# declare-lab/tango

Hardware: AMD Instinct MI355X
Metric: audio-seconds generated/sec, Tango-full 200-step, batch=32, guidance=3 (higher is better)
Workload: dtype fp16; 1 GPU; BASELINE config 3: Tango-full UNet (866M) 200-step DDPM CFG=3 denoise + mel-VAE decode + HiFi-GAN, 32 prompts/GPU x 64 tokens; global_batch=32, text_len=64, denoise_steps=200, parallelism=dp1, rccl_ranks=1, hipgraph=True, fp8_attention=False

## Files before the change

include/tango_engine.h:

```cpp
#ifndef TANGO_ENGINE_H
#define TANGO_ENGINE_H

#include <stdint.h>

#ifdef __cplusplus
extern "C" {
#endif

#define TANGO_DTYPE_F32 0
#define TANGO_DTYPE_F16 1
#define TANGO_DTYPE_BF16 2

#define TANGO_PRED_EPSILON 0
#define TANGO_PRED_SAMPLE 1
#define TANGO_PRED_V 2

#define TANGO_RULE_DDPM 0
#define TANGO_RULE_DDIM 1
#define TANGO_RULE_DPM_MULTISTEP 2

#define TANGO_MAX_LEVELS 8

typedef struct tango_engine tango_engine_t;

// ... 36 lines not shown
  int32_t unet_attn_fp8;
} tango_config_t;

typedef struct tango_denoise_args {
  float* latents;
  const float* prompt_embeds;
  const uint8_t* prompt_mask;
  int32_t batch;
  int32_t text_len;
  int32_t num_steps;
  const int64_t* timesteps;
  const float* coef;
  float guidance_scale;
  int32_t prediction_type;
  int32_t rule;
  int32_t clip_sample;
  float clip_sample_range;
  const float* noise;
  uint64_t seed;
  int32_t sample_offset;
  int32_t use_graph;
  const float* beat_embeds;
  const uint8_t* beat_mask;
  int32_t beat_len;
  const float* chord_embeds;
  const uint8_t* chord_mask;
  int32_t chord_len;
  const uint8_t* prompt_mask_host;
  int32_t coef_width;
  const float* known_latents;
  const float* latent_mask;
  const float* blend_coef;
  const float* blend_noise;
} tango_denoise_args_t;

const char* tango_last_error(void);
const char* tango_version(void);

int tango_engine_create(const tango_config_t* cfg, tango_engine_t** out);
void tango_engine_destroy(tango_engine_t* h);

int tango_engine_num_weights(tango_engine_t* h);
const char* tango_engine_weight_name(tango_engine_t* h, int i);
int tango_engine_set_weight(tango_engine_t* h, const char* name, const float* dev_ptr, const int64_t* shape, int ndim);
int tango_engine_finalize_weights(tango_engine_t* h);

int tango_engine_denoise(tango_engine_t* h, const tango_denoise_args_t* args, void* stream);

int tango_engine_unet_forward(tango_engine_t* h, const float* sample, int64_t timestep, const float* prompt_embeds,
                              const uint8_t* prompt_mask, float* out, int batch2, int text_len, void* stream);

int tango_engine_unet_forward_music(tango_engine_t* h, const float* sample, int64_t timestep, const float* prompt_embeds,
                                    const uint8_t* prompt_mask, const float* beat_embeds, const uint8_t* beat_mask,
                                    const float* chord_embeds, const uint8_t* chord_mask, float* out, int batch2, int text_len,
                                    int beat_len, int chord_len, void* stream);

int tango_engine_vae_decode(tango_engine_t* h, const float* latents, float* mel, int batch, void* stream);
int tango_engine_vae_encode(tango_engine_t* h, const float* mel, float* moments, int batch, void* stream);
int tango_engine_vocode(tango_engine_t* h, const float* mel, int16_t* wav, int batch, int mel_frames, int* n_samples, void* stream);
int tango_engine_vocoder_samples(tango_engine_t* h, int mel_frames);

int tango_engine_encode_text(tango_engine_t* h, const int64_t* input_ids, const uint8_t* attention_mask, float* out, int batch,
                             int text_len, void* stream);

int tango_engine_mel_frames(tango_engine_t* h, int n_samples);
int tango_engine_mel_spectrogram(tango_engine_t* h, const float* wav, float* mel, float* log_magnitudes, float* energy, int batch,
                                 int n_samples, int* n_frames, void* stream);

int tango_engine_last_denoise_ms(tango_engine_t* h, float* total_ms, float* per_step_ms);
int tango_engine_last_step_gflop(tango_engine_t* h, double* gflop);

int tango_engine_set_plan_budget(tango_engine_t* h, uint64_t bytes);
int tango_engine_plan_stats(tango_engine_t* h, uint64_t* bytes_in_use, int* plans);
int tango_engine_drop_plans(tango_engine_t* h);

int tango_engine_profile_unet(tango_engine_t* h, int batch2, int text_len, char* report, int report_cap, void* stream);
int tango_engine_profile_vae(tango_engine_t* h, int batch, char* report, int report_cap, void* stream);
int tango_engine_profile_vocoder(tango_engine_t* h, int batch, int frames, char* report, int report_cap, void* stream);
void tango_tuning_reload(void);
const char* tango_debug_linear_route(int dtype, int M, int N, int K, int geglu, int ln_fold, int residual, int vt);

int tango_op_conv2d(int dtype, const float* x, const float* w, const float* bias, float* out, int B, int Cin, int H, int W,
                    int Cout, int stride, int upsample, void* stream);
int tango_op_linear(int dtype, const float* x, const float* w, const float* bias, const float* residual, float* out, int M,
                    int N, int K, int a_act, int e_act, int geglu, void* stream);
int tango_op_linear_ln(int dtype, const float* x, const float* w, const float* bias, const float* gamma, const float* beta,
                       const float* residual, float* out, int M, int N, int K, int geglu, float eps, void* stream);
int tango_op_linear_qkv(int dtype, const float* x, const float* w, const float* gamma, const float* beta, float* out_qk,
                        float* out_vt, int B, int S, int C, int K, float eps, void* stream);
int tango_op_linear_qkv_perm(int dtype, const float* x, const float* w, const float* gamma, const float* beta, float* out_qk,
                             float* out_vt, int B, int S, int C, int K, float eps, int vt_perm, void* stream);
int tango_op_ff_fused(int dtype, const float* x, const float* w1, const float* b1, const float* gamma, const float* beta, const float* w2,
                      const float* b2, float* out, int M, int C, int H, float eps, int mode, int reps, float* ms_out, void* stream);
int tango_op_qkv_stat(int dtype, const float* x, const float* w, const float* gamma, const float* beta, float* out_qk, float* out_vt, int B,
                      int S, int C, float eps, int mode, int reps, float* ms_out, void* stream);
int tango_op_conv1d(int dtype, const float* x, const float* w, const float* bias, const float* residual, float* out, int B,
                    int Cin, int L, int Cout, int k, int dilation, int a_act, float a_slope, int e_act, float e_slope, void* stream);
int tango_op_conv_transpose1d(int dtype, const float* x, const float* w, const float* bias, float* out, int B, int Cin, int L,
                              int Cout, int k, int stride, int padding, int a_act, float a_slope, void* stream);
int tango_op_groupnorm(int dtype, const float* x, const float* gamma, const float* beta, float* out, int B, int C, int HW,
                       int groups, float eps, int act, void* stream);
int tango_op_layernorm(int dtype, const float* x, const float* gamma, const float* beta, float* out, int rows, int C, float eps,
                       void* stream);
int tango_op_attention(int dtype, const float* q, const float* k, const float* v, const float* bias, float* out, int B, int heads,
                       int Sq, int Skv, float scale, void* stream);
int tango_op_attention_ex(int dtype, const float* q, const float* k, const float* v, const float* bias, float* out, int B, int heads,
                          int Sq, int Skv, float scale, int flags, void* stream);
int tango_op_xattn_block(int dtype, const float* x, const float* gamma, const float* beta, const float* wq, const float* k, const float* v,
                         const float* bias, const float* wo, const float* bo, float* out, int B, int HW, int L, float eps, void* stream);
int tango_op_sched_step(float* latents, const float* model_out_nchw, const float* noise, const float* coef8, int B, int C, int HW,
                        int cfg, float guidance, int pred_type, int rule, int clip, float clip_range, void* stream);

int tango_op_sched_multistep(float* latents, const float* model_out_nchw, float* ring, const float* coef16, int step, int B, int C,
                             int HW, int cfg, float guidance, int pred_type, int algo, void* stream);

int tango_op_philox_normal(float* out, int B, int C, int HW, int step, uint64_t seed, int sample_offset, void* stream);

int tango_op_sched_masked(float* latents, const float* model_out_nchw, const float* noise, float* ring, const float* coef, int coef_width,
                          int step, int num_steps, const float* known_latents, const float* latent_mask, const float* blend_coef,
                          const float* blend_noise, uint64_t seed, int sample_offset, int B, int C, int HW, int cfg, float guidance,
                          int pred_type, int rule, void* stream);

int tango_op_philox_normal_blend(float* out, int B, int C, int HW, int step, uint64_t seed, int sample_offset, void* stream);

#ifdef __cplusplus
}
#endif
#endif
```

tango_amd/_lib.py:

```python
import ctypes as C
import os

_HERE = os.path.dirname(os.path.abspath(__file__))
LIB_PATH = os.path.join(_HERE, "lib", "libtango_hip.so")
MAX_LEVELS = 8

DTYPES = {"fp32": 0, "float32": 0, "f32": 0, "fp16": 1, "float16": 1, "f16": 1, "bf16": 2, "bfloat16": 2}
PRED = {"epsilon": 0, "sample": 1, "v_prediction": 2}
RULE = {"ddpm": 0, "ddim": 1, "dpmsolver": 2}


class TangoConfig(C.Structure):
    _fields_ = [
        ("dtype", C.c_int32),
        ("unet_levels", C.c_int32),
        ("unet_channels", C.c_int32 * MAX_LEVELS),
        ("unet_heads", C.c_int32 * MAX_LEVELS),
        ("unet_cross_attn", C.c_int32 * MAX_LEVELS),
        ("unet_layers_per_block", C.c_int32),
        ("unet_in_channels", C.c_int32),
        ("unet_out_channels", C.c_int32),
        ("unet_cross_dim", C.c_int32),
        ("unet_groups", C.c_int32),
        ("unet_eps", C.c_float),
        ("unet_flip_sin_to_cos", C.c_int32),
        ("unet_freq_shift", C.c_float),
        ("latent_h", C.c_int32),
        ("latent_w", C.c_int32),
        ("vae_levels", C.c_int32),
        ("vae_ch", C.c_int32),
        ("vae_ch_mult", C.c_int32 * MAX_LEVELS),
        ("vae_num_res_blocks", C.c_int32),
        ("vae_z_channels", C.c_int32),
        ("vae_embed_dim", C.c_int32),
        ("vae_out_ch", C.c_int32),
        ("vae_scale_factor", C.c_float),
        ("voc_n_ups", C.c_int32),
        ("voc_rates", C.c_int32 * MAX_LEVELS),
        ("voc_kernels", C.c_int32 * MAX_LEVELS),
        ("voc_initial_channel", C.c_int32),
        ("voc_num_mels", C.c_int32),
        ("voc_n_resblocks", C.c_int32),
        ("voc_res_kernels", C.c_int32 * 4),
        ("voc_res_dilations", (C.c_int32 * 4) * 4),
        ("t5_layers", C.c_int32),
        ("t5_d_model", C.c_int32),
        ("t5_d_kv", C.c_int32),
        ("t5_heads", C.c_int32),
        ("t5_d_ff", C.c_int32),
        ("t5_vocab", C.c_int32),
        ("t5_rel_buckets", C.c_int32),
        ("t5_rel_max_distance", C.c_int32),
        ("t5_eps", C.c_float),
        ("vae_encoder", C.c_int32),
        ("vae_in_channels", C.c_int32),
        ("stft_filter_length", C.c_int32),
        ("stft_hop_length", C.c_int32),
        ("stft_n_mel", C.c_int32),
        ("unet_music", C.c_int32),
        ("unet_attn_fp8", C.c_int32),
    ]


class DenoiseArgs(C.Structure):
    _fields_ = [
        ("latents", C.c_void_p),
        ("prompt_embeds", C.c_void_p),
        ("prompt_mask", C.c_void_p),
        ("batch", C.c_int32),
        ("text_len", C.c_int32),
        ("num_steps", C.c_int32),
        ("timesteps", C.c_void_p),
        ("coef", C.c_void_p),
        ("guidance_scale", C.c_float),
        ("prediction_type", C.c_int32),
        ("rule", C.c_int32),
        ("clip_sample", C.c_int32),
        ("clip_sample_range", C.c_float),
        ("noise", C.c_void_p),
        ("seed", C.c_uint64),
        ("sample_offset", C.c_int32),
        ("use_graph", C.c_int32),
        ("beat_embeds", C.c_void_p),
        ("beat_mask", C.c_void_p),
        ("beat_len", C.c_int32),
        ("chord_embeds", C.c_void_p),
        ("chord_mask", C.c_void_p),
        ("chord_len", C.c_int32),
        ("prompt_mask_host", C.c_void_p),
        ("coef_width", C.c_int32),
        ("known_latents", C.c_void_p),
        ("latent_mask", C.c_void_p),
        ("blend_coef", C.c_void_p),
        ("blend_noise", C.c_void_p),
    ]


SYMBOLS = [
    "tango_last_error", "tango_version", "tango_tuning_reload", "tango_debug_linear_route", "tango_engine_create", "tango_engine_destroy",
    "tango_engine_num_weights", "tango_engine_weight_name", "tango_engine_set_weight",
    "tango_engine_finalize_weights", "tango_engine_denoise", "tango_engine_unet_forward", "tango_engine_unet_forward_music",
    "tango_engine_vae_decode", "tango_engine_vae_encode", "tango_engine_vocode", "tango_engine_vocoder_samples", "tango_engine_encode_text",
    "tango_engine_mel_frames", "tango_engine_mel_spectrogram",
    "tango_engine_last_denoise_ms", "tango_engine_last_step_gflop", "tango_engine_profile_unet", "tango_engine_profile_vae", "tango_engine_profile_vocoder", "tango_engine_set_plan_budget", "tango_engine_plan_stats", "tango_engine_drop_plans", "tango_op_conv2d", "tango_op_linear", "tango_op_linear_ln", "tango_op_ff_fused", "tango_op_qkv_stat", "tango_op_linear_qkv", "tango_op_linear_qkv_perm", "tango_op_conv1d",
    "tango_op_conv_transpose1d", "tango_op_groupnorm", "tango_op_layernorm", "tango_op_attention", "tango_op_attention_ex", "tango_op_xattn_block",
    "tango_op_sched_step", "tango_op_sched_multistep", "tango_op_philox_normal",
    "tango_op_sched_masked", "tango_op_philox_normal_blend",
]

_lib = None


def load():
    global _lib
    if _lib is not None:
        return _lib
    if not os.path.exists(LIB_PATH):
        raise ImportError(
            "tango_amd: %s not found. Build it with `make -C tango_amd/csrc` "
            "(or __graft_entry__.build()); the engine has no CPU/PyTorch fallback." % LIB_PATH)
    lib = C.CDLL(LIB_PATH, mode=C.RTLD_GLOBAL)
    vp, ci, cf, i64 = C.c_void_p, C.c_int, C.c_float, C.c_int64
    lib.tango_last_error.restype = C.c_char_p
    lib.tango_version.restype = C.c_char_p
    lib.tango_tuning_reload.restype = None
    lib.tango_engine_create.argtypes = [C.POINTER(TangoConfig), C.POINTER(vp)]
    lib.tango_engine_destroy.argtypes = [vp]
    lib.tango_engine_destroy.restype = None
    lib.tango_engine_num_weights.argtypes = [vp]
    lib.tango_engine_weight_name.argtypes = [vp, ci]
    lib.tango_engine_weight_name.restype = C.c_char_p
    lib.tango_engine_set_weight.argtypes = [vp, C.c_char_p, vp, C.POINTER(i64), ci]
    lib.tango_engine_finalize_weights.argtypes = [vp]
    lib.tango_engine_denoise.argtypes = [vp, C.POINTER(DenoiseArgs), vp]
    lib.tango_engine_unet_forward.argtypes = [vp, vp, i64, vp, vp, vp, ci, ci, vp]
    lib.tango_engine_unet_forward_music.argtypes = [vp, vp, i64, vp, vp, vp, vp, vp, vp, vp, ci, ci, ci, ci, vp]
    lib.tango_engine_vae_decode.argtypes = [vp, vp, vp, ci, vp]
    lib.tango_engine_vae_encode.argtypes = [vp, vp, vp, ci, vp]
    lib.tango_engine_vocode.argtypes = [vp, vp, vp, ci, ci, C.POINTER(ci), vp]
    lib.tango_engine_vocoder_samples.argtypes = [vp, ci]
    lib.tango_engine_encode_text.argtypes = [vp, vp, vp, vp, ci, ci, vp]
    lib.tango_engine_mel_frames.argtypes = [vp, ci]
    lib.tango_engine_mel_spectrogram.argtypes = [vp, vp, vp, vp, vp, ci, ci, C.POINTER(ci), vp]
    lib.tango_engine_last_denoise_ms.argtypes = [vp, C.POINTER(cf), C.POINTER(cf)]
    lib.tango_engine_last_step_gflop.argtypes = [vp, C.POINTER(C.c_double)]
    lib.tango_engine_profile_unet.argtypes = [vp, ci, ci, C.c_char_p, ci, vp]
    lib.tango_engine_profile_vae.argtypes = [vp, ci, C.c_char_p, ci, vp]
    lib.tango_engine_profile_vocoder.argtypes = [vp, ci, ci, C.c_char_p, ci, vp]
    lib.tango_engine_set_plan_budget.argtypes = [vp, C.c_uint64]
    lib.tango_engine_drop_plans.argtypes = [vp]
    lib.tango_debug_linear_route.argtypes = [ci] * 8
    lib.tango_debug_linear_route.restype = C.c_char_p
    lib.tango_engine_plan_stats.argtypes = [vp, C.POINTER(C.c_uint64), C.POINTER(ci)]
    lib.tango_op_conv2d.argtypes = [ci, vp, vp, vp, vp, ci, ci, ci, ci, ci, ci, ci, vp]
    lib.tango_op_linear.argtypes = [ci, vp, vp, vp, vp, vp, ci, ci, ci, ci, ci, ci, vp]
    lib.tango_op_linear_ln.argtypes = [ci, vp, vp, vp, vp, vp, vp, vp, ci, ci, ci, ci, cf, vp]
    lib.tango_op_ff_fused.argtypes = [ci, vp, vp, vp, vp, vp, vp, vp, vp, ci, ci, ci, cf, ci, ci, vp, vp]
    lib.tango_op_qkv_stat.argtypes = [ci, vp, vp, vp, vp, vp, vp, ci, ci, ci, cf, ci, ci, vp, vp]
    lib.tango_op_linear_qkv.argtypes = [ci, vp, vp, vp, vp, vp, vp, ci, ci, ci, ci, cf, vp]
    lib.tango_op_linear_qkv_perm.argtypes = [ci, vp, vp, vp, vp, vp, vp, ci, ci, ci, ci, cf, ci, vp]
    lib.tango_op_conv1d.argtypes = [ci, vp, vp, vp, vp, vp, ci, ci, ci, ci, ci, ci, ci, cf, ci, cf, vp]
    lib.tango_op_conv_transpose1d.argtypes = [ci, vp, vp, vp, vp, ci, ci, ci, ci, ci, ci, ci, ci, cf, vp]
    lib.tango_op_groupnorm.argtypes = [ci, vp, vp, vp, vp, ci, ci, ci, ci, cf, ci, vp]
    lib.tango_op_layernorm.argtypes = [ci, vp, vp, vp, vp, ci, ci, cf, vp]
    lib.tango_op_attention.argtypes = [ci, vp, vp, vp, vp, vp, ci, ci, ci, ci, cf, vp]
    lib.tango_op_attention_ex.argtypes = [ci, vp, vp, vp, vp, vp, ci, ci, ci, ci, cf, ci, vp]
    lib.tango_op_xattn_block.argtypes = [ci, vp, vp, vp, vp, vp, vp, vp, vp, vp, vp, ci, ci, ci, cf, vp]
    lib.tango_op_sched_step.argtypes = [vp, vp, vp, vp, ci, ci, ci, ci, cf, ci, ci, ci, cf, vp]
    lib.tango_op_sched_multistep.argtypes = [vp, vp, vp, vp, ci, ci, ci, ci, ci, cf, ci, ci, vp]
    lib.tango_op_philox_normal.argtypes = [vp, ci, ci, ci, ci, C.c_uint64, ci, vp]
    lib.tango_op_philox_normal_blend.argtypes = [vp, ci, ci, ci, ci, C.c_uint64, ci, vp]
    lib.tango_op_sched_masked.argtypes = [vp, vp, vp, vp, vp, ci, ci, ci, vp, vp, vp, vp, C.c_uint64, ci, ci, ci, ci, ci, cf, ci, ci, vp]
    _lib = lib
    return lib


def check(rc, what="tango engine call"):
    if rc != 0:
        msg = load().tango_last_error()
        msg = msg.decode() if msg else "unknown error"
        if "cannot be larger" in msg or "unknown prediction" in msg:
            raise ValueError(msg)
        raise RuntimeError("%s failed: %s" % (what, msg))
```

tango_amd/csrc/common.h:

```cpp
#pragma once
#include <hip/hip_runtime.h>
#include <stdint.h>
#include <string>

namespace tango {

enum DType : int { DT_F32 = 0, DT_F16 = 1, DT_BF16 = 2 };

typedef _Float16 f16;
typedef __bf16 bf16;
typedef float f32x4 __attribute__((ext_vector_type(4)));
typedef float f32x2 __attribute__((ext_vector_type(2)));
typedef _Float16 f16x8 __attribute__((ext_vector_type(8)));
typedef _Float16 f16x4 __attribute__((ext_vector_type(4)));
typedef __bf16 bf16x8 __attribute__((ext_vector_type(8)));
typedef __bf16 bf16x4 __attribute__((ext_vector_type(4)));
typedef unsigned u32x4 __attribute__((ext_vector_type(4)));
typedef unsigned u32x2 __attribute__((ext_vector_type(2)));

inline size_t dtype_size(int dt) { return dt == DT_F32 ? 4 : 2; }

template <typename T> struct TypeTag;
template <> struct TypeTag<float> { static constexpr int dt = DT_F32; };
template <> struct TypeTag<f16> { static constexpr int dt = DT_F16; };
// ... 26 lines not shown
template <typename T> __device__ __forceinline__ float to_f(T v) { return (float)v; }
template <typename T> __device__ __forceinline__ T from_f(float v) { return (T)v; }

__device__ __forceinline__ float silu_f(float x) { return x / (1.0f + __expf(-x)); }
__device__ __forceinline__ float gelu_erf_f(float x) { return 0.5f * x * (1.0f + erff(x * 0.70710678118654752440f)); }
__device__ __forceinline__ float gelu_tanh_f(float x) {
  return 0.5f * x * (1.0f + tanhf(0.7978845608028654f * (x + 0.044715f * x * x * x)));
}
typedef float f32x2_t __attribute__((ext_vector_type(2)));
__device__ __forceinline__ f32x2_t gelu_erf_poly2(const f32x2_t x) {
  f32x2_t xc;
  xc.x = __builtin_amdgcn_fmed3f(x.x, -4.25f, 4.25f);
  xc.y = __builtin_amdgcn_fmed3f(x.y, -4.25f, 4.25f);
  const f32x2_t t = xc * xc;
  f32x2_t q = f32x2_t{1.498029197e-11f, 1.498029197e-11f} + t * 1.123676848e-12f;
  q = __builtin_elementwise_fma(q, t, f32x2_t{-7.180728823e-09f, -7.180728823e-09f});
  q = __builtin_elementwise_fma(q, t, f32x2_t{3.825664002e-07f, 3.825664002e-07f});
  q = __builtin_elementwise_fma(q, t, f32x2_t{-1.045047183e-05f, -1.045047183e-05f});
  q = __builtin_elementwise_fma(q, t, f32x2_t{1.811638670e-04f, 1.811638670e-04f});
  q = __builtin_elementwise_fma(q, t, f32x2_t{-2.193588131e-03f, -2.193588131e-03f});
  q = __builtin_elementwise_fma(q, t, f32x2_t{1.957916536e-02f, 1.957916536e-02f});
  q = __builtin_elementwise_fma(q, t, f32x2_t{-1.326353318e-01f, -1.326353318e-01f});
  q = __builtin_elementwise_fma(q, t, f32x2_t{7.977887478e-01f, 7.977887478e-01f});
  const f32x2_t e = q * xc, h = x * 0.5f;
  return __builtin_elementwise_fma(h, e, h);
}
template <typename T, typename V4> __device__ __forceinline__ void glu_gate4(V4& v, const float g[4], int tanh_form) {
  if (tanh_form) {
#pragma unroll
    for (int r = 0; r < 4; ++r) v[r] = v[r] * gelu_tanh_f(g[r]);
  } else if constexpr (sizeof(T) == 4) {
#pragma unroll
    for (int r = 0; r < 4; ++r) v[r] = v[r] * gelu_erf_f(g[r]);
  } else {
    const f32x2_t a = gelu_erf_poly2(f32x2_t{g[0], g[1]}), b = gelu_erf_poly2(f32x2_t{g[2], g[3]});
    v[0] = v[0] * a.x; v[1] = v[1] * a.y; v[2] = v[2] * b.x; v[3] = v[3] * b.y;
  }
}

enum Act : int { ACT_NONE = 0, ACT_SILU = 1, ACT_LRELU = 2, ACT_GELU = 3, ACT_TANH = 4, ACT_GELU_TANH = 5 };

__device__ __forceinline__ float apply_act(float x, int act, float slope) {
  switch (act) {
    case ACT_SILU: return silu_f(x);
    case ACT_LRELU: return x > 0.f ? x : x * slope;
    case ACT_GELU: return gelu_erf_f(x);
    case ACT_TANH: return tanhf(x);
    case ACT_GELU_TANH: return gelu_tanh_f(x);
    default: return x;
  }
}

template <typename V4> __device__ __forceinline__ void apply_act4(V4& v, int act, float slope) {
  if (act == ACT_LRELU) {
#pragma unroll
    for (int r = 0; r < 4; ++r) v[r] = v[r] > 0.f ? v[r] : v[r] * slope;
  } else if (act == ACT_SILU) {
#pragma unroll
    for (int r = 0; r < 4; ++r) v[r] = silu_f(v[r]);
  } else if (act == ACT_TANH) {
#pragma unroll
    for (int r = 0; r < 4; ++r) v[r] = tanhf(v[r]);
  } else if (act == ACT_GELU) {
#pragma unroll
    for (int r = 0; r < 4; ++r) v[r] = gelu_erf_f(v[r]);
  } else if (act == ACT_GELU_TANH) {
#pragma unroll
    for (int r = 0; r < 4; ++r) v[r] = gelu_tanh_f(v[r]);
  }
}

struct View {
  void* p = nullptr;
  int64_t ld = 0;
  int C = 0;
};

enum GatherMode : int { GATHER_1D = 0, GATHER_2D = 1 };
enum Epi : int { EPI_NONE = 0, EPI_GEGLU = 1, EPI_I16 = 2, EPI_VT = 3 };

struct GemmParams {
  const void* A = nullptr;
  const void* W = nullptr;
  const float* bias = nullptr;
  const float* bias2 = nullptr;
  const int* step_ptr = nullptr;
  int bias2_stride = 0;
  const void* R = nullptr;
  int64_t ldr = 0;
  void* out = nullptr;
  int64_t ldo = 0;
  int out_f32 = 0;
  int M = 0, N = 0, K = 0, Cin = 0;
  int64_t Kp = 0;
  int64_t lda = 0;
  int stage_epi = 0;
  int mode = GATHER_1D;
  int H = 0, Wd = 0, Hin = 0, Win = 0, stride = 1, ups = 0;
  int pad = 1;
  int rows_pb = 0, Lin = 0, taps = 1, tap_step = 1, in_off = 0, in_mul = 1;
  int Lout = 0, out_mul = 1, out_off = 0;
  int a_act = ACT_NONE;
  float a_slope = 0.f;
  int epi = EPI_NONE;
  int glu_tanh = 0;
  int e_act = ACT_NONE;
  float e_slope = 0.f;
  float alpha = 1.f;
  float out_scale = 1.f;
  int bias_rows = 0;
  void* vt = nullptr;
  int vt_n0 = 0, vt_S = 1;
  int64_t vt_ld = 0;
  int vt_perm = 0;
  const float* rowvec = nullptr;
  int64_t rowvec_rows = 0;
  int rowvec_per = 1;
  void* out_lo = nullptr;
  int64_t ldo_lo = 0;
  int64_t wb_stride = 0;
  int wb_rows = 0;
  int ln_fold = 0;
  float ln_eps = 1e-5f;
  const float* wsum = nullptr;
  const float* row_stats = nullptr;
  int splitk = 1;
  float* ws = nullptr;
  int batch = 1;
  int64_t sA = 0, sW = 0, sO = 0, sR = 0, sBias = 0;
};

int launch_gemm(int dtype, const GemmParams& p, hipStream_t s);
enum GemmRoute : int { ROUTE_NONE = 0, ROUTE_WIDE, ROUTE_STREAM, ROUTE_CONV_WIDE, ROUTE_CONV_HALO, ROUTE_DMA, ROUTE_TILE, ROUTE_DUO };
int gemm_route(int dtype, const GemmParams& p);
bool gemm_rowvec_ok(int dtype, const GemmParams& p);
bool conv_halo_ok(int dtype, const GemmParams& p);
int launch_conv_halo(int dtype, const GemmParams& p, const unsigned char* zero_page, hipStream_t s);
bool gemm_wide_ok(int dtype, const GemmParams& p);
int launch_gemm_wide(int dtype, const GemmParams& p, hipStream_t s);
int gemm_wide_pers_cus();
bool gemm_duo_ok(int dtype, const GemmParams& p);
int launch_gemm_duo(int dtype, const GemmParams& p, hipStream_t s);
inline bool gemm_ln_fold_ok(int dtype, const GemmParams& p);
bool conv_wide_ok(int dtype, const GemmParams& p);
int launch_conv_wide(int dtype, const GemmParams& p, const unsigned char* zero_page, hipStream_t s);
int conv_wide_pick_splitk(int dtype, const GemmParams& p);
int launch_splitk_reduce(int dtype, const GemmParams& p, hipStream_t s);
bool gemm_dma_ok(int dtype, const GemmParams& p);
int launch_gemm_dma(int dtype, const GemmParams& p, const unsigned char* zero_page, hipStream_t s);
int gemm_init();
int gemm_pick_splitk(int dtype, const GemmParams& p);
bool linear_stream_ok(int dtype, const GemmParams& p);
int launch_linear_stream(int dtype, const GemmParams& p, hipStream_t s);
inline bool gemm_ln_fold_ok(int dtype, const GemmParams& p) { return linear_stream_ok(dtype, p) || gemm_wide_ok(dtype, p) || gemm_duo_ok(dtype, p); }
int launch_fold_ln(int dtype, const void* W, int64_t Kp, const float* gamma, const float* beta, const float* bias_in, void* Wo,
                   float* bias_out, float* wsum, int N, int K, hipStream_t s);

struct FFParams {
  const void* x = nullptr; int64_t ldx = 0;
  const void* w1 = nullptr; int64_t ld1 = 0;
  const float* b1 = nullptr;
  const void* w2 = nullptr; int64_t ld2 = 0;
  const float* b2 = nullptr;
  void* out = nullptr; int64_t ldo = 0;
  int M = 0, C = 0, H = 0;
  float eps = 1e-5f;
  int plain_loop = 0;
};
bool ff_fused_ok(int dtype, const FFParams& p);
int launch_ff_fused(int dtype, const FFParams& p, hipStream_t s);

struct QKVParams {
  const void* x = nullptr; int64_t ldx = 0;
  const void* w = nullptr; int64_t ldw = 0;
  const float* b = nullptr;
  void* out = nullptr; int64_t ldo = 0;
  void* vt = nullptr; int64_t vt_ld = 0; int vt_S = 0;
  int vt_perm = 0;
  int M = 0, N = 0, K = 0, n_rm = 0;
  int ln = 1; float eps = 1e-5f;
  const float* gstats = nullptr;
  int groups = 0, rows_ps = 0;
};
bool qkv_stat_ok(int dtype, const QKVParams& p);
int launch_qkv_stat(int dtype, const QKVParams& p, hipStream_t s);

struct GroupNormParams {
  const void* x; int64_t ldx;
  void* y; int64_t ldy;
  const float* gamma; const float* beta;
  int B, rows, C, groups;
  float eps;
  int act;
  float* partial;
  float* scale_shift;
  unsigned* sync = nullptr;
};
constexpr int COOP_SYNC_SLOTS = 1024;
constexpr int coop_sync_words() { return 2 * COOP_SYNC_SLOTS + 16; }
size_t groupnorm_ws_floats(int B, int rows, int C, int groups);
int launch_gn_stats_fold(int dtype, const GroupNormParams& p, const void* W, int64_t Kp, const float* bias, int N, void* Wf, float* bf, hipStream_t s);
bool gn_fold_ok(int dtype, const GroupNormParams& p, int N);
bool gn_stats_mr_ok(int dtype, const GroupNormParams& p);
int launch_gn_stats_mr(int dtype, const GroupNormParams& p, float* mr, hipStream_t s);
int launch_groupnorm(int dtype, const GroupNormParams& p, hipStream_t s);

int launch_layernorm(int dtype, const void* x, int64_t ldx, void* y, int64_t ldy, const float* gamma,
                     const float* beta, int rows, int C, float eps, hipStream_t s);
int launch_ln_stats(int dtype, const void* x, int64_t ldx, float* stats, int rows, int C, float eps, hipStream_t s);

struct AttnParams {
  const void* q; int64_t ldq;
  const void* k; int64_t ldk;
  const void* vt; int64_t ldvt;
  void* o; int64_t ldo;
  const float* bias;
  const float* pos_bias = nullptr;
  int B, heads, Sq, Skv;
  float scale;
  int vt_perm = 0;
  int fp8_pv = 0;
};
int launch_attention(int dtype, const AttnParams& p, hipStream_t s);
__host__ __device__ inline int vt_perm_pos(int s) { return (s & ~31) | ((s & 12) << 1) | ((s & 16) >> 2) | (s & 3); }
bool attention_vt_perm_ok(int dtype, const AttnParams& p);

struct XAttnParams {
  const void* x; int64_t ldx;
  const void* wq;
// ... 76 lines not shown
```

tango_amd/csrc/conv_wide.hip:

```cpp
#include <cstdlib>
#include <type_traits>

#include "common.h"
#include "tuning.h"
#include "gemm_device.h"
#include "gemm_wide_device.h"

namespace tango {

static constexpr int CW_HALO_MAX = 544;
static constexpr int CW_NA_WIDE = 5;
static constexpr int CW_NA = CW_NA_WIDE;
static constexpr int CW_HALO_MAX_TALL = 800;
static constexpr int CW_NA_TALL = 7;

template <typename T, bool RES, bool SK, int SCH, bool TALL>
__global__ __launch_bounds__(512) void conv3x3_wide_kernel(const GemmParams p, const unsigned char* zero_page, const int SR, const int nseg,
                                                           const int abytes, const int prio) {
  constexpr int BM = TALL ? 512 : 256, BN = TALL ? 160 : 320, CB = 64, NST = 4;
  constexpr int CW_NA = TALL ? CW_NA_TALL : CW_NA_WIDE;
  constexpr int BK = CB / (int)sizeof(T);
  constexpr int WST = BN * CB;
  constexpr int WRG = BN / 16;
  constexpr int WRGW = (WRG + 7) / 8;
  constexpr int TM = 4, TN = 10;
  extern __shared__ __attribute__((aligned(16))) unsigned char dsm[];
  unsigned char* const As = dsm;
  unsigned char* const Ws = dsm + 2 * abytes;

  const int NT = p.N / BN;
  int bid = blockIdx.x;
  {
    const int nblk = gridDim.x, q = nblk >> 3, r = nblk & 7, xcd = bid & 7, idx = bid >> 3;
    bid = (xcd < r ? xcd * (q + 1) : r * (q + 1) + (xcd - r) * q) + idx;
  }
  const int m0 = (bid / NT) * BM, n0 = (bid % NT) * BN;
  const unsigned char* Ab = (const unsigned char*)p.A;
  const unsigned char* Wb = (const unsigned char*)p.W;
  const int tid = threadIdx.x, lane = tid & 63;
  const int wave = __builtin_amdgcn_readfirstlane(tid >> 6);
  const int wm = TALL ? wave : wave & 3, wn = TALL ? 0 : wave >> 2;
  const int lrow = lane >> 2, slot = lane & 3;

  const int H = p.H, Wd = p.Wd, hw = H * Wd;
  const int HW2 = Wd + 2, SEG = (SR + 2) * HW2;
  const int HALO = nseg * SEG, HALO_RG = (HALO + 15) >> 4;
  const int b0 = m0 / hw;
  const int y0 = nseg == 1 ? (m0 - b0 * hw) / Wd : 0;

  unsigned* const aoff_lds = (unsigned*)(Ws + NST * WST) + tid;
#pragma unroll
  for (int t = 0; t < CW_NA; ++t) {
    unsigned off = ~0u;
    const int h = ((t * 8 + wave) << 4) + lrow;
    if (h < HALO) {
      const int seg = h / SEG, rem = h - seg * SEG;
      const int hy = rem / HW2, hx = rem - hy * HW2;
      const int y = y0 + hy - 1, x = hx - 1;
      const int pc = slot ^ ((h >> 1) & 2);
      if ((unsigned)y < (unsigned)H && (unsigned)x < (unsigned)Wd)
        off = (unsigned)(((((int64_t)(b0 + seg) * p.Hin + (y >> p.ups)) * p.Win + (x >> p.ups)) * p.lda) * (int64_t)sizeof(T) + pc * 16);
    }
    aoff_lds[t * 512] = off;
  }
  const int wrow_d = wave * 16 + lrow;
  const unsigned w_off0_init = (unsigned)(((int64_t)wrow_d * p.Kp) * (int64_t)sizeof(T) + ((slot ^ ((wrow_d >> 1) & 2)) * 16));
  aoff_lds[CW_NA * 512] = w_off0_init;
  const unsigned w_step = (unsigned)(128 * p.Kp * (int64_t)sizeof(T));
  const unsigned char* const Wt = Wb + (int64_t)n0 * p.Kp * (int64_t)sizeof(T);
  const int my_w = wave < WRG - 8 * (WRGW - 1) ? WRGW : WRGW - 1;

  auto issue_a_off = [&](const int t, const int cc, const int buf, const unsigned off) {
    const unsigned char* src = off != ~0u ? Ab + (int64_t)cc * CB + off : zero_page;
    __builtin_amdgcn_global_load_lds((gptr_t)src, (lptr_t)(As + buf * abytes + (t * 8 + wave) * 1024), 16, 0, 0);
  };
  auto issue_a = [&](const int t, const int cc, const int buf) {
    if (t * 8 + wave < HALO_RG) issue_a_off(t, cc, buf, aoff_lds[t * 512]);
  };
  auto issue_w_one = [&](const int i, int koff, const int st, const unsigned w_off0) {
    const int rg = wave + 8 * i;
    if (rg < WRG) {
      asm volatile("" : "+s"(koff));
      const unsigned char* base = Wt + koff;
      unsigned o = w_off0 + i * w_step;
      asm volatile("" : "+v"(o));
      __builtin_amdgcn_global_load_lds((gptr_t)(base + o), (lptr_t)(Ws + st * WST + rg * 1024), 16, 0, 0);
    }
  };
  auto issue_w = [&](const int tap, const int cc, const int st) {
    const int koff = (tap * p.Cin + cc * BK) * (int)sizeof(T);
    const unsigned w_off0 = aoff_lds[CW_NA * 512];
#pragma unroll
    for (int i = 0; i < WRGW; ++i) issue_w_one(i, koff, st, w_off0);
  };
  auto wait_n = [&](const int n) {
    switch (n) {
      case 0: wait_vmcnt_lit<0>(); break;
      case 1: wait_vmcnt_lit<1>(); break;
      case 2: wait_vmcnt_lit<2>(); break;
      case 3: wait_vmcnt_lit<3>(); break;
      case 4: wait_vmcnt_lit<4>(); break;
      case 5: wait_vmcnt_lit<5>(); break;
      case 6: wait_vmcnt_lit<6>(); break;
      case 7: wait_vmcnt_lit<7>(); break;
      default: wait_vmcnt_lit<8>(); break;
    }
  };

  f32x4 acc[TN][TM];
#pragma unroll
  for (int a = 0; a < TN; ++a)
#pragma unroll
    for (int b = 0; b < TM; ++b) acc[a][b] = f32x4{0.f, 0.f, 0.f, 0.f};

  int h0 = 0, hd[TM];
#pragma unroll
  for (int b = 0; b < TM; ++b) {
    const int pm = wm * 64 + b * 16 + (lane & 15);
    const int seg = pm / hw, r = pm - seg * hw;
    const int ly = r / Wd, x = r - ly * Wd;
    const int hb_ = seg * SEG + ly * HW2 + x;
    if (b == 0) h0 = hb_;
    hd[b] = __builtin_amdgcn_readfirstlane(hb_ - h0);
  }
  const int kg = lane >> 4;
  const int wrow0 = wn * (TN * 16) + (lane & 15);
  const int wfoff = wrow0 * CB + ((kg ^ ((wrow0 >> 1) & 2)) << 4);

  int cc0 = 0, cc1 = p.Cin / BK;
  if (SK) {
    const int per = (cc1 + (int)gridDim.y - 1) / (int)gridDim.y;
    cc0 = (int)blockIdx.y * per;
    cc1 = cc1 < cc0 + per ? cc1 : cc0 + per;
  }
  const int NI = (cc1 - cc0) * 9;

  const int half = wave >> 2;
#pragma unroll
  for (int t = 0; t < CW_NA; ++t) issue_a(t, cc0, cc0 & 1);
  issue_w(0, cc0, 0);
  issue_w(1, cc0, 1);
  issue_w(2, cc0, 2);
  wait_n(2 * my_w);
  pp_barrier();
  if (half) pp_barrier();
  if (prio == 2 && half) __builtin_amdgcn_s_setprio(1);
  int st = 0, item = 0;
  int prev_h = 0;
  unsigned hoff = 0u;
  unsigned w_off0 = w_off0_init;
  asm volatile("" : "+v"(w_off0));
  for (int cc = cc0; cc < cc1; ++cc) {
    const unsigned char* Ah = As + (cc & 1) * abytes;
    const bool more_c = cc + 1 < cc1;
#pragma unroll 1
    for (int tap = 0; tap < 9; ++tap, ++item) {
      const unsigned char* Wst = Ws + st * WST;
      const int toff = (tap / 3) * HW2 + (tap % 3);
      const bool iss_h = more_c && tap < CW_NA && tap * 8 + wave < HALO_RG;
      const bool iss_w = item + 3 < NI;
      const int st3 = st == 0 ? 3 : st - 1;
      int koff3;
      {
        int t3 = tap + 3, c3 = cc;
        if (t3 >= 9) { t3 -= 9; c3 = cc + 1; }
        koff3 = (t3 * p.Cin + c3 * BK) * (int)sizeof(T);
      }
      if (SCH != 0) { if (iss_h) hoff = aoff_lds[tap * 512]; }
      u32x4 wf[TN], xf[TM];
#pragma unroll
      for (int a = 0; a < TN; ++a) wf[a] = *(const u32x4*)(Wst + wfoff + a * 16 * CB);
#pragma unroll
      for (int b = 0; b < TM; ++b) {
        int hs = hd[b] + toff;
        asm volatile("" : "+s"(hs));
        const int h = h0 + hs;
        xf[b] = *(const u32x4*)(Ah + h * CB + ((kg ^ ((h >> 1) & 2)) << 4));
      }
      if (item + 1 < NI) wait_n(prev_h + (item + 2 < NI ? my_w : 0));
      prev_h = iss_h ? 1 : 0;
      pp_barrier();
      if (SCH == 0) {
        if (more_c && tap < CW_NA) issue_a(tap, cc + 1, (cc + 1) & 1);
        const int t3 = tap + 3;
        if (t3 < 9) issue_w(t3, cc, st3);
        else if (more_c) issue_w(t3 - 9, cc + 1, st3);
      }
      if (prio == 0) __builtin_amdgcn_s_setprio(1);
#pragma unroll
      for (int a = 0; a < TN; ++a) {
#pragma unroll
        for (int b = 0; b < TM; ++b) Mma<T>::run(acc[a][b], wf[a], xf[b]);
        if (SCH != 0 && (a & 1) == 0 && (a >> 1) <= WRGW) {
          const int sl = a >> 1;
          __builtin_amdgcn_sched_barrier(0);
          if (sl == 0) { if (iss_h) issue_a_off(tap, cc + 1, (cc + 1) & 1, hoff); }
          else if (iss_w) issue_w_one(sl - 1, koff3, st3, w_off0);
          __builtin_amdgcn_sched_barrier(0);
        }
      }
      if (prio == 0) __builtin_amdgcn_s_setprio(0);
      pp_barrier();
      st = st == NST - 1 ? 0 : st + 1;
    }
  }
  if (!half) pp_barrier();
  if (prio == 2) __builtin_amdgcn_s_setprio(0);
  __syncthreads();
  unsigned char* const slice = dsm + wave * (WIDE_STAGE_BYTES + 1280);
  if (SK) {
    wide_epilogue_raw(p, acc, (int)blockIdx.y, m0 + wm * 64, n0 + wn * (TN * 16), lane, slice);
    return;
  }
  const float mean[TM] = {0.f, 0.f, 0.f, 0.f}, rstd[TM] = {1.f, 1.f, 1.f, 1.f};
  wide_epilogue<T, false, RES, false>(p, acc, mean, rstd, m0 + wm * 64, n0 + wn * (TN * 16), lane, slice);
}

template <int OFF> __device__ __forceinline__ void cwp_lds_read(u32x4& v, const unsigned base) {
  asm volatile("ds_read_b128 %0, %1 offset:%2" : "=v"(v) : "v"(base), "n"(OFF));
}
__device__ __forceinline__ void cwp_lds_wait_all(u32x4 (&wf)[10], u32x4 (&xf)[4], unsigned& hoff) {
  asm volatile("s_waitcnt lgkmcnt(0)"
               : "+v"(wf[0]), "+v"(wf[1]), "+v"(wf[2]), "+v"(wf[3]), "+v"(wf[4]), "+v"(wf[5]), "+v"(wf[6]), "+v"(wf[7]), "+v"(wf[8]), "+v"(wf[9]),
                 "+v"(xf[0]), "+v"(xf[1]), "+v"(xf[2]), "+v"(xf[3]), "+v"(hoff));
}
__device__ __forceinline__ void cwp_lds_read_b32(unsigned& v, const unsigned addr) { asm volatile("ds_read_b32 %0, %1" : "=v"(v) : "v"(addr)); }
template <int I, int N, typename F> __device__ __forceinline__ void cwp_for(F&& f) {
  if constexpr (I < N) { f(std::integral_constant<int, I>{}); cwp_for<I + 1, N>(f); }
}

template <typename T, bool RES, bool SK, int MODE = 0>
__global__ __launch_bounds__(512) void conv3x3_wide_pipe_kernel(const GemmParams p, const unsigned char* zero_page, const int SR, const int nseg,
                                                                const int abytes, const int prio) {
  constexpr bool LOCK = MODE == 1, SKEW = MODE == 2;
  constexpr int BM = 256, BN = 320, CB = 64, NST = 4;
  constexpr int BK = CB / (int)sizeof(T);
  constexpr int WST = BN * CB;
  constexpr int WRG = BN / 16;
  constexpr int WRGW = (WRG + 7) / 8;
  constexpr int TM = 4, TN = 10;
  extern __shared__ __attribute__((aligned(16))) unsigned char dsm[];
  unsigned char* const As = dsm;
  unsigned char* const Ws = dsm + 2 * abytes;

  const int NT = p.N / BN;
  int bid = blockIdx.x;
  {
    const int nblk = gridDim.x, q = nblk >> 3, r = nblk & 7, xcd = bid & 7, idx = bid >> 3;
    bid = (xcd < r ? xcd * (q + 1) : r * (q + 1) + (xcd - r) * q) + idx;
  }
  const int m0 = (bid / NT) * BM, n0 = (bid % NT) * BN;
  const unsigned char* Ab = (const unsigned char*)p.A;
  const unsigned char* Wb = (const unsigned char*)p.W;
  const int tid = threadIdx.x, lane = tid & 63;
  const int wave = __builtin_amdgcn_readfirstlane(tid >> 6);
  const int wm = wave & 3, wn = wave >> 2;
  const int lrow = lane >> 2, slot = lane & 3;

  const int H = p.H, Wd = p.Wd, hw = H * Wd;
  const int HW2 = Wd + 2, SEG = (SR + 2) * HW2;
  const int HALO = nseg * SEG, HALO_RG = (HALO + 15) >> 4;
  const int b0 = m0 / hw;
  const int y0 = nseg == 1 ? (m0 - b0 * hw) / Wd : 0;

  unsigned* const aoff_lds = (unsigned*)(Ws + NST * WST) + tid;
#pragma unroll
  for (int t = 0; t < CW_NA; ++t) {
    unsigned off = ~0u;
    const int h = ((t * 8 + wave) << 4) + lrow;
    if (h < HALO) {
      const int seg = h / SEG, rem = h - seg * SEG;
      const int hy = rem / HW2, hx = rem - hy * HW2;
      const int y = y0 + hy - 1, x = hx - 1;
      const int pc = slot ^ ((h >> 1) & 2);
      if ((unsigned)y < (unsigned)H && (unsigned)x < (unsigned)Wd)
        off = (unsigned)(((((int64_t)(b0 + seg) * p.Hin + (y >> p.ups)) * p.Win + (x >> p.ups)) * p.lda) * (int64_t)sizeof(T) + pc * 16);
    }
    aoff_lds[t * 512] = off;
  }
  const int wrow_d = wave * 16 + lrow;
  const unsigned w_off0_init = (unsigned)(((int64_t)wrow_d * p.Kp) * (int64_t)sizeof(T) + ((slot ^ ((wrow_d >> 1) & 2)) * 16));
  const unsigned w_step = (unsigned)(128 * p.Kp * (int64_t)sizeof(T));
  const unsigned char* const Wt = Wb + (int64_t)n0 * p.Kp * (int64_t)sizeof(T);
  const int my_w = wave < WRG - 8 * (WRGW - 1) ? WRGW : WRGW - 1;

  auto issue_a_off = [&](const int t, const int cc, const int buf, const unsigned off) {
    const unsigned char* src = off != ~0u ? Ab + (int64_t)cc * CB + off : zero_page;
    __builtin_amdgcn_global_load_lds((gptr_t)src, (lptr_t)(As + buf * abytes + (t * 8 + wave) * 1024), 16, 0, 0);
  };
  auto issue_w_one = [&](const int i, int koff, const int st, const unsigned w_off0) {
    const int rg = wave + 8 * i;
    if (rg < WRG) {
      asm volatile("" : "+s"(koff));
      const unsigned char* base = Wt + koff;
      unsigned o = w_off0 + i * w_step;
      asm volatile("" : "+v"(o));
      __builtin_amdgcn_global_load_lds((gptr_t)(base + o), (lptr_t)(Ws + st * WST + rg * 1024), 16, 0, 0);
    }
// ... 173 lines not shown
    unsigned xa[TM];
#pragma unroll
    for (int b = 0; b < TM; ++b) xa[b] = MORE1 ? xaddr(b, buf1, toff1) : 0u;
    cwp_for<0, TM>([&](auto b_tag) {
      constexpr int b = decltype(b_tag)::value;
      Mma<T>::run(acc[9][b], wf[9], xf[b]);
      __builtin_amdgcn_sched_barrier(0);
      if (MORE1) cwp_lds_read<0>(xf[b], xa[b]);
      if constexpr (2 + b <= WRGW) { if (half) dma_slot(std::integral_constant<int, 2 + b>{}); }
      __builtin_amdgcn_sched_barrier(0);
    });
    if (MORE1) {
      cwp_lds_read<9 * 16 * CB>(wf[9], wsrc);
      cwp_lds_read_b32(hoff, aoff_addr + (unsigned)(tap1 < CW_NA ? tap1 : 0) * 2048u);
      cwp_lds_wait_all(wf, xf, hoff);
    }
    return iss_h ? 1 : 0;
  };
  auto run_items = [&](auto item_fn) __attribute__((always_inline)) {
    int tap = 0, cc = cc0, prev_h = 0;
    unsigned hoff = hoff0;
#pragma unroll 1
    for (int item = 0; item + 1 < NI; ++item) {
      prev_h = item_fn(std::true_type{}, item, tap, cc, prev_h, hoff);
      if (tap == 8) { tap = 0; ++cc; } else ++tap;
    }
    item_fn(std::false_type{}, NI - 1, 8, cc1 - 1, prev_h, hoff);
  };
  if constexpr (SKEW) run_items(do_item_skew);
  else run_items(do_item);
  if (MODE == 0 && !half) pp_barrier();
  if (prio == 2) __builtin_amdgcn_s_setprio(0);
  __syncthreads();
  unsigned char* const slice = dsm + wave * (WIDE_STAGE_BYTES + 1280);
  if (SK) {
    wide_epilogue_raw(p, acc, (int)blockIdx.y, m0 + wm * 64, n0 + wn * (TN * 16), lane, slice);
    return;
  }
  const float mean[TM] = {0.f, 0.f, 0.f, 0.f}, rstd[TM] = {1.f, 1.f, 1.f, 1.f};
  wide_epilogue<T, false, RES, false>(p, acc, mean, rstd, m0 + wm * 64, n0 + wn * (TN * 16), lane, slice);
}

struct WideHaloGeom {
  int SR, nseg, halo;
};

static bool wide_halo_geom(const GemmParams& p, WideHaloGeom& g, const int BM = 256) {
  const int hw = p.H * p.Wd;
  if (p.Wd <= 0 || BM % p.Wd != 0) return false;
  if (hw >= BM) {
    if (hw % BM != 0) return false;
    g.SR = BM / p.Wd; g.nseg = 1;
  } else {
    if (BM % hw != 0) return false;
    g.SR = p.H; g.nseg = BM / hw;
  }
  g.halo = g.nseg * (g.SR + 2) * (p.Wd + 2);
  if (!((16 % p.Wd == 0 || p.Wd % 16 == 0) && hw % 16 == 0)) return false;
  return g.halo <= (BM == 512 ? CW_HALO_MAX_TALL : CW_HALO_MAX);
}

static bool conv_wide_tall_ok(const GemmParams& p) {
  if (!tuning().conv_tall || p.splitk > 1 || p.M % 512 != 0) return false;
  WideHaloGeom g;
  return wide_halo_geom(p, g, 512);
}

bool conv_wide_ok(int dtype, const GemmParams& p) {
  if (tuning().no_wide_conv || dtype == DT_F32) return false;
  if (p.mode != GATHER_2D || p.stride != 1 || p.pad != 1 || p.ups < 0 || p.ups > 1 || (p.Hin << p.ups) != p.H || (p.Win << p.ups) != p.Wd) return false;
  if (p.batch != 1 || p.a_act != ACT_NONE || p.epi != EPI_NONE || p.bias_rows) return false;
  if (p.splitk > 1 ? (!p.ws || p.splitk > p.Cin / 32 || p.N % 4 != 0) : (p.e_act != ACT_NONE || p.out_f32)) return false;
  if ((p.Cin * 2) % 64 != 0 || p.K != 9 * p.Cin || p.M % 256 != 0 || p.N % 320 != 0) return false;
  if (p.ldo % 8 != 0 || ((uintptr_t)p.out & 15) || (p.R && (p.ldr % 8 != 0 || ((uintptr_t)p.R & 15)))) return false;
  if ((p.lda * 2) % 16 != 0 || (p.Kp * 2) % 16 != 0 || ((uintptr_t)p.A & 15) || ((uintptr_t)p.W & 15)) return false;
  if (((uintptr_t)p.bias & 15) || ((uintptr_t)p.bias2 & 15) || (p.bias2 && p.bias2_stride % 4 != 0)) return false;
  if ((int64_t)(p.M >> (2 * p.ups)) * p.lda * 2 >= (int64_t)0xFFFF0000 || (int64_t)320 * p.Kp * 2 >= (int64_t)0xFFFF0000) return false;
  WideHaloGeom g;
  if (!wide_halo_geom(p, g)) return false;
  const long tiles = (long)(p.M / 256) * (p.N / 320) * (p.splitk > 1 ? p.splitk : 1);
  return tuning().force_big_kernels || tiles >= 224;
}

int conv_wide_pick_splitk(int dtype, const GemmParams& p) {
  GemmParams q = p;
  q.splitk = 1;
  if (tuning().force_big_kernels || p.mode != GATHER_2D || dtype == DT_F32 || p.M % 256 != 0 || p.N % 320 != 0 || p.Cin % 32 != 0) return 0;
  const long tiles = (long)(p.M / 256) * (p.N / 320);
  if (tiles > 96 || tiles < 16) return 0;
  int s = (int)((256 + tiles / 2) / tiles);
  const int nc = p.Cin / 32;
  if (s > nc / 4) s = nc / 4;
  if (s < 2) return 0;
  float dummy_ws = 0.f;
  q.splitk = s; q.ws = &dummy_ws;
  return conv_wide_ok(dtype, q) ? s : 0;
}

template <typename T, bool RES, bool SK, int SCH, bool TALL = false>
static int launch_conv_wide_sch(const GemmParams& p, const unsigned char* zero_page, hipStream_t s) {
  constexpr int BM = TALL ? 512 : 256, BN = TALL ? 160 : 320, NA = TALL ? CW_NA_TALL : CW_NA_WIDE;
  WideHaloGeom g;
  if (!wide_halo_geom(p, g, BM)) TANGO_FAIL("conv_wide: unsupported geometry");
  const int abytes = ((g.halo + 15) / 16) * 1024;
  int lds = 2 * abytes + 4 * BN * 64 + (NA + 1) * 512 * 4;
  const int epi_lds = 8 * (WIDE_STAGE_BYTES + 1280);
  if (lds < epi_lds) lds = epi_lds;
  auto kfn = conv3x3_wide_kernel<T, RES, SK, SCH, TALL>;
  TANGO_TRY(ensure_dyn_lds(reinterpret_cast<const void*>(kfn), lds));
  const int tiles = (p.M / BM) * (p.N / BN);
  hipLaunchKernelGGL(kfn, dim3((unsigned)tiles, (unsigned)(p.splitk > 1 ? p.splitk : 1)), dim3(512), lds, s, p, zero_page, g.SR, g.nseg, abytes, tuning().wide_prio);
  TANGO_HIP(hipGetLastError());
  if (p.splitk > 1) TANGO_TRY(launch_splitk_reduce(TypeTag<T>::dt, p, s));
  return 0;
}

template <typename T, bool RES, bool SK>
static int launch_conv_wide_pipe(const GemmParams& p, const unsigned char* zero_page, hipStream_t s) {
  WideHaloGeom g;
  if (!wide_halo_geom(p, g)) TANGO_FAIL("conv_wide: unsupported geometry");
  const int abytes = ((g.halo + 15) / 16) * 1024;
  int lds = 2 * abytes + 4 * 320 * 64 + (CW_NA + 1) * 512 * 4;
  const int epi_lds = 8 * (WIDE_STAGE_BYTES + 1280);
  if (lds < epi_lds) lds = epi_lds;
  const int mode = tuning().conv_pipe;
  auto kfn = mode == 3 ? conv3x3_wide_pipe_kernel<T, RES, SK, 2> : mode == 2 ? conv3x3_wide_pipe_kernel<T, RES, SK, 1> : conv3x3_wide_pipe_kernel<T, RES, SK, 0>;
  TANGO_TRY(ensure_dyn_lds(reinterpret_cast<const void*>(kfn), lds));
  const int tiles = (p.M / 256) * (p.N / 320);
  hipLaunchKernelGGL(kfn, dim3((unsigned)tiles, (unsigned)(p.splitk > 1 ? p.splitk : 1)), dim3(512), lds, s, p, zero_page, g.SR, g.nseg, abytes, tuning().wide_prio);
  TANGO_HIP(hipGetLastError());
  if (p.splitk > 1) TANGO_TRY(launch_splitk_reduce(TypeTag<T>::dt, p, s));
  return 0;
}

template <typename T, bool RES, bool SK = false>
static int launch_conv_wide_cfg(const GemmParams& p, const unsigned char* zero_page, hipStream_t s) {
  if (tuning().conv_pipe && !(SK ? false : conv_wide_tall_ok(p))) return launch_conv_wide_pipe<T, RES, SK>(p, zero_page, s);
  if constexpr (!SK) {
    if (conv_wide_tall_ok(p)) return launch_conv_wide_sch<T, RES, false, 1, true>(p, zero_page, s);
  }
  switch (tuning().wide_sched) {
    case 0: return launch_conv_wide_sch<T, RES, SK, 0>(p, zero_page, s);
    default: return launch_conv_wide_sch<T, RES, SK, 1>(p, zero_page, s);
  }
}

int launch_conv_wide(int dtype, const GemmParams& p, const unsigned char* zero_page, hipStream_t s) {
  if (!zero_page) TANGO_FAIL("conv_wide: gemm_init() was not called (zero page for the LDS-DMA gather)");
  switch (dtype) {
    case DT_F16:
      if (p.splitk > 1) return launch_conv_wide_cfg<f16, false, true>(p, zero_page, s);
      return p.R ? launch_conv_wide_cfg<f16, true>(p, zero_page, s) : launch_conv_wide_cfg<f16, false>(p, zero_page, s);
    case DT_BF16:
      if (p.splitk > 1) return launch_conv_wide_cfg<bf16, false, true>(p, zero_page, s);
      return p.R ? launch_conv_wide_cfg<bf16, true>(p, zero_page, s) : launch_conv_wide_cfg<bf16, false>(p, zero_page, s);
  }
  TANGO_FAIL("conv_wide: 16-bit dtypes only");
}

}
```

tango_amd/csrc/elementwise.hip:

```cpp
#include "common.h"

namespace tango {

__device__ __forceinline__ void philox4x32(unsigned c0, unsigned c1, unsigned c2, unsigned c3, unsigned k0, unsigned k1,
                                           unsigned* out) {
#pragma unroll
  for (int r = 0; r < 10; ++r) {
    const unsigned long long p0 = (unsigned long long)0xD2511F53u * c0;
    const unsigned long long p1 = (unsigned long long)0xCD9E8D57u * c2;
    const unsigned n0 = (unsigned)(p1 >> 32) ^ c1 ^ k0;
    const unsigned n1 = (unsigned)p1;
    const unsigned n2 = (unsigned)(p0 >> 32) ^ c3 ^ k1;
    const unsigned n3 = (unsigned)p0;
    c0 = n0; c1 = n1; c2 = n2; c3 = n3;
    k0 += 0x9E3779B9u; k1 += 0xBB67AE85u;
  }
  out[0] = c0; out[1] = c1; out[2] = c2; out[3] = c3;
}

__device__ __forceinline__ void box_muller(unsigned a, unsigned b, float& n0, float& n1) {
  const float u1 = ((float)a + 1.0f) * 2.3283064365386963e-10f;
  const float u2 = (float)b * 2.3283064365386963e-10f;
  const float r = sqrtf(-2.0f * __logf(u1));
  float s, c;
// ... 372 lines not shown
                    float slope, hipStream_t s) {
  const int epv = dtype == DT_F32 ? 4 : 8;
  if (n % epv) TANGO_FAIL("avg3: n must be a multiple of the 16-byte vector");
  const int64_t nvec = n / epv;
  unsigned nb = (unsigned)((nvec + 255) / 256);
  if (nb > 8192) nb = 8192;
  switch (dtype) {
    case DT_F32: hipLaunchKernelGGL((avg3_act_kernel<float>), dim3(nb), dim3(256), 0, s, (const float*)a, (const float*)b, (const float*)c, (float*)y, nvec, scale, act, slope); break;
    case DT_F16: hipLaunchKernelGGL((avg3_act_kernel<f16>), dim3(nb), dim3(256), 0, s, (const f16*)a, (const f16*)b, (const f16*)c, (f16*)y, nvec, scale, act, slope); break;
    case DT_BF16: hipLaunchKernelGGL((avg3_act_kernel<bf16>), dim3(nb), dim3(256), 0, s, (const bf16*)a, (const bf16*)b, (const bf16*)c, (bf16*)y, nvec, scale, act, slope); break;
    default: TANGO_FAIL("avg3: bad dtype");
  }
  TANGO_HIP(hipGetLastError());
  return 0;
}

__global__ void mask_bias_kernel(const uint8_t* __restrict__ m, float* __restrict__ bias, int n) {
  const int i = blockIdx.x * 256 + threadIdx.x;
  if (i < n) bias[i] = (1.0f - (m[i] ? 1.0f : 0.0f)) * -10000.0f;
}
int launch_mask_bias(const uint8_t* mask, float* bias, int n, hipStream_t s) {
  hipLaunchKernelGGL(mask_bias_kernel, dim3((unsigned)((n + 255) / 256)), dim3(256), 0, s, mask, bias, n);
  TANGO_HIP(hipGetLastError());
  return 0;
}

__global__ void timestep_embedding_kernel(const int64_t* __restrict__ ts, float* __restrict__ out, int n, int dim, int flip,
                                          float freq_shift) {
  const int i = blockIdx.x, half = dim / 2;
  for (int j = threadIdx.x; j < half; j += blockDim.x) {
    const float ex = __fdiv_rn(__fmul_rn(-9.210340371976184f, (float)j), (float)half - freq_shift);
    const float arg = __fmul_rn((float)ts[i], expf(ex));
    const float sv = sinf(arg), cv = cosf(arg);
    if (flip) { out[(int64_t)i * dim + j] = cv; out[(int64_t)i * dim + half + j] = sv; }
    else { out[(int64_t)i * dim + j] = sv; out[(int64_t)i * dim + half + j] = cv; }
  }
  if ((dim & 1) && threadIdx.x == 0) out[(int64_t)i * dim + dim - 1] = 0.f;
}
int launch_timestep_embedding(const int64_t* ts_dev, float* out, int n, int dim, int flip, float freq_shift, hipStream_t s) {
  hipLaunchKernelGGL(timestep_embedding_kernel, dim3((unsigned)n), dim3(256), 0, s, ts_dev, out, n, dim, flip, freq_shift);
  TANGO_HIP(hipGetLastError());
  return 0;
}

__device__ __forceinline__ int geglu_row(int o, int half) {
  const int j = o < half ? o : o - half;
  return 32 * (j >> 4) + (j & 15) + (o < half ? 0 : 16);
}

template <typename T>
__global__ __launch_bounds__(256) void pack_kernel(const float* __restrict__ src, T* __restrict__ dst, int O, int Tn, int I,
                                                   int64_t so, int64_t st, int64_t si, int64_t Kp, int64_t row_off, int perm) {
  const int64_t idx = (int64_t)blockIdx.x * 256 + threadIdx.x;
  if (idx >= (int64_t)O * Kp) return;
  const int o = (int)(idx / Kp);
  const int k = (int)(idx - (int64_t)o * Kp);
  float v = 0.f;
  if (k < Tn * I) {
    const int t = k / I, i = k - t * I;
    v = src[(int64_t)o * so + (int64_t)t * st + (int64_t)i * si];
  }
  int orow = o;
  if (perm == 1) orow = geglu_row(o, O / 2);
  else if (perm == 2) orow = 32 * (o >> 4) + (o & 15);
  else if (perm == 3) orow = 32 * (o >> 4) + (o & 15) + 16;
  dst[(row_off + orow) * Kp + k] = from_f<T>(v);
}

int launch_pack(int dtype, const float* src, void* dst, int O, int Tn, int I, int64_t so, int64_t st, int64_t si, int64_t Kp,
                int64_t dst_row_off, hipStream_t s) {
  const int perm = dst_row_off < 0 ? (int)(-dst_row_off) : 0;
  const int64_t ro = perm ? 0 : dst_row_off;
  const unsigned nb = (unsigned)(((int64_t)O * Kp + 255) / 256);
  switch (dtype) {
    case DT_F32: hipLaunchKernelGGL((pack_kernel<float>), dim3(nb), dim3(256), 0, s, src, (float*)dst, O, Tn, I, so, st, si, Kp, ro, perm); break;
    case DT_F16: hipLaunchKernelGGL((pack_kernel<f16>), dim3(nb), dim3(256), 0, s, src, (f16*)dst, O, Tn, I, so, st, si, Kp, ro, perm); break;
    case DT_BF16: hipLaunchKernelGGL((pack_kernel<bf16>), dim3(nb), dim3(256), 0, s, src, (bf16*)dst, O, Tn, I, so, st, si, Kp, ro, perm); break;
    default: TANGO_FAIL("pack: bad dtype");
  }
  TANGO_HIP(hipGetLastError());
  return 0;
}


template <typename T>
__global__ __launch_bounds__(256) void pointwise_small_kernel(const float* __restrict__ src, const float* __restrict__ W,
                                                              const float* __restrict__ bias, T* __restrict__ dst, int64_t ld,
                                                              int B, int Cin, int Cout, int HW, float scale) {
  const int64_t idx = (int64_t)blockIdx.x * 256 + threadIdx.x;
  if (idx >= (int64_t)B * HW) return;
  const int b = (int)(idx / HW), hw = (int)(idx - (int64_t)b * HW);
  float x[16];
  for (int c = 0; c < Cin; ++c) x[c] = src[((int64_t)b * Cin + c) * HW + hw] * scale;
  for (int o = 0; o < Cout; ++o) {
    float a = bias ? bias[o] : 0.f;
    for (int c = 0; c < Cin; ++c) a += W[o * Cin + c] * x[c];
    dst[idx * ld + o] = from_f<T>(a);
  }
}
int launch_pointwise_small(int dtype, const float* src, const float* W, const float* b, void* dst, int64_t ld, int B, int Cin,
                           int Cout, int HW, float scale, hipStream_t s) {
  if (Cin > 16) TANGO_FAIL("pointwise_small: Cin > 16");
  const unsigned nb = (unsigned)(((int64_t)B * HW + 255) / 256);
  switch (dtype) {
    case DT_F32: hipLaunchKernelGGL((pointwise_small_kernel<float>), dim3(nb), dim3(256), 0, s, src, W, b, (float*)dst, ld, B, Cin, Cout, HW, scale); break;
    case DT_F16: hipLaunchKernelGGL((pointwise_small_kernel<f16>), dim3(nb), dim3(256), 0, s, src, W, b, (f16*)dst, ld, B, Cin, Cout, HW, scale); break;
    case DT_BF16: hipLaunchKernelGGL((pointwise_small_kernel<bf16>), dim3(nb), dim3(256), 0, s, src, W, b, (bf16*)dst, ld, B, Cin, Cout, HW, scale); break;
    default: TANGO_FAIL("pointwise_small: bad dtype");
  }
  TANGO_HIP(hipGetLastError());
  return 0;
}

__global__ __launch_bounds__(256) void pointwise_out_nchw_kernel(const float* __restrict__ src, int64_t ld, const float* __restrict__ W,
                                                                 const float* __restrict__ bias, float* __restrict__ dst, int B, int Cin,
                                                                 int Cout, int HW) {
  const int64_t idx = (int64_t)blockIdx.x * 256 + threadIdx.x;
  if (idx >= (int64_t)B * HW) return;
  const int b = (int)(idx / HW), hw = (int)(idx - (int64_t)b * HW);
  float x[32];
  for (int c = 0; c < Cin; ++c) x[c] = src[idx * ld + c];
  for (int o = 0; o < Cout; ++o) {
    float a = bias ? bias[o] : 0.f;
    for (int c = 0; c < Cin; ++c) a += W[o * Cin + c] * x[c];
    dst[((int64_t)b * Cout + o) * HW + hw] = a;
  }
}
int launch_pointwise_out_nchw(const float* src, int64_t ld, const float* W, const float* b, float* dst, int B, int Cin, int Cout, int HW,
                              hipStream_t s) {
  if (Cin > 32) TANGO_FAIL("pointwise_out_nchw: Cin > 32");
  const unsigned nb = (unsigned)(((int64_t)B * HW + 255) / 256);
  hipLaunchKernelGGL(pointwise_out_nchw_kernel, dim3(nb), dim3(256), 0, s, src, ld, W, b, dst, B, Cin, Cout, HW);
  TANGO_HIP(hipGetLastError());
  return 0;
}

__global__ void permute_geglu_bias_kernel(const float* __restrict__ src, float* __restrict__ dst, int n) {
  const int i = blockIdx.x * 256 + threadIdx.x;
  if (i < n) dst[geglu_row(i, n / 2)] = src[i];
}
int launch_permute_geglu_bias(const float* src, float* dst, int n, hipStream_t s) {
  hipLaunchKernelGGL(permute_geglu_bias_kernel, dim3((unsigned)((n + 255) / 256)), dim3(256), 0, s, src, dst, n);
  TANGO_HIP(hipGetLastError());
  return 0;
}

int launch_fill_zero(void* p, size_t bytes, hipStream_t s) {
  TANGO_HIP(hipMemsetAsync(p, 0, bytes, s));
  return 0;
}

int launch_linear_f32(const float*, const float*, const float*, float*, int, int, int, int, int, hipStream_t) {
  TANGO_FAIL("linear_f32: not implemented (use launch_gemm with DT_F32)");
}

template <typename T>
__global__ __launch_bounds__(256) void embed_gather_kernel(const int64_t* __restrict__ ids, const float* __restrict__ table,
                                                           T* __restrict__ out, int64_t ld, int rows, int D, int vocab) {
  const int r = blockIdx.x;
  int64_t id = ids[r];
  id = id < 0 ? 0 : (id >= vocab ? vocab - 1 : id);
  const float* src = table + id * D;
  T* dst = out + (int64_t)r * ld;
  for (int c = threadIdx.x * 4; c < D; c += 1024) {
    const f32x4 v = *(const f32x4*)(src + c);
    dst[c] = from_f<T>(v[0]); dst[c + 1] = from_f<T>(v[1]); dst[c + 2] = from_f<T>(v[2]); dst[c + 3] = from_f<T>(v[3]);
// ... 143 lines not shown
```

tango_amd/csrc/engine.h:

```cpp
#pragma once
#include <array>
#include <functional>
#include <map>
#include <memory>
#include <string>
#include <unordered_map>
#include <vector>

#include "../../include/tango_engine.h"
#include "common.h"

namespace tango {

using Op = std::function<int(hipStream_t)>;

struct Program {
  std::vector<Op> ops;
  std::vector<std::string> labels;
  std::vector<double> flops;
  int run(hipStream_t s) const {
    for (const auto& o : ops) TANGO_TRY(o(s));
    return 0;
  }
  int run_profiled(hipStream_t s, std::string& report) const;
};

struct Arena {
  char* base = nullptr;
  size_t off = 0, peak = 0;
  void* alloc(size_t bytes) {
    off = (off + 255) & ~(size_t)255;
    void* p = base ? (void*)(base + off) : (void*)(uintptr_t)(0x1000 + off);
    off += bytes;
    if (off > peak) peak = off;
    return p;
  }
  size_t mark() const { return off; }
  void release(size_t m) { off = m; }
};

struct TView {
  void* p = nullptr;
  int64_t ld = 0;
  int C = 0;
};

struct WMat {
  void* W = nullptr;
  float* b = nullptr;
  int N = 0, K = 0, Cin = 0, taps = 1;
  int64_t Kp = 0;
  bool im2col = false;
  void* Wln = nullptr;
  float* bln = nullptr;
  float* wsum = nullptr;
};
struct WNorm {
  float* g = nullptr;
  float* b = nullptr;
  int C = 0;
  float eps = 1e-5f;
};
struct WLinF32 {
  float* W = nullptr;
  float* b = nullptr;
  int N = 0, K = 0;
};

struct ResW {
  int cin = 0, cout = 0;
  WNorm n1, n2;
  WMat c1, c2, sc;
  bool has_sc = false;
  bool has_temb = false;
  WLinF32 temb;
  float* temb_table = nullptr;
};
struct XfW {
  int C = 0, heads = 0;
  int cond = 0;
  WNorm gn, ln1, ln2, ln3;
  WMat proj_in, qkv, o1, q2, kv2, o2, ff1, ff2, proj_out;
  void* q2p = nullptr;
  float* bq2p = nullptr;
  float* wsum2p = nullptr;
};
struct VaeAttnW {
  WNorm gn;
  WMat qk, v, proj;
};
struct ConvTW {
  int cin = 0, cout = 0, k = 0, u = 0, pad = 0;
  std::vector<WMat> phase;
  float* b = nullptr;
};
struct VocResW {
  int ch = 0, k = 0;
  std::vector<int> dil;
  std::vector<WMat> c1, c2;
};

struct Slot {
  std::string name;
  std::vector<int64_t> shape;
  bool set = false;
  std::function<int(const float*, hipStream_t)> pack;
};

struct PlanMeta {
  size_t bytes = 0;
  uint64_t stamp = 0;
};

struct UNetPlan {
  PlanMeta meta;
  int B2 = 0, L = 0;
  int Lc[3] = {0, 0, 0};
  char* slab = nullptr;
  Program pre, step;
  void* xin = nullptr;
  float* eps = nullptr;
  void* enc = nullptr;
  float* bias = nullptr;
  void* encs[3] = {nullptr, nullptr, nullptr};
  float* biases[3] = {nullptr, nullptr, nullptr};
  int n_short = 0;
  int* key0 = nullptr;
  hipGraph_t graph = nullptr;
  hipGraphExec_t exec = nullptr;
  hipGraph_t graph_k = nullptr;
  hipGraphExec_t exec_k = nullptr;
  int k_steps = 0;
  hipGraph_t graph_ms = nullptr;
  hipGraphExec_t exec_ms = nullptr;
  hipGraph_t graph_k_ms = nullptr;
// ... 8 lines not shown
  void* ext_xin = nullptr;
  float* ext_eps = nullptr;
  bool cfg_shared = false;
  unsigned* sync = nullptr;
};
struct T5LayerW {
  WNorm ln1, ln2;
  WMat qkv, o, wi, wo;
};
struct T5Plan {
  PlanMeta meta;
  int B = 0, L = 0;
  char* slab = nullptr;
  Program prog;
  int64_t* ids = nullptr;
  float* bias = nullptr;
  int* bucket = nullptr;
  float* pos_bias = nullptr;
  float* out = nullptr;
};
struct VaePlan {
  PlanMeta meta;
  int B = 0;
  char* slab = nullptr;
  Program prog;
  void* in = nullptr;
  void* out = nullptr;
  size_t in_bytes = 0, out_bytes = 0;
  int n_out = 0;
};

struct StftPlan {
  PlanMeta meta;
  int B = 0, N = 0, T = 0, Np = 0, Kp2 = 0, ldz = 0;
  char* slab = nullptr;
  float *in = nullptr, *xpad = nullptr, *Z = nullptr, *mag = nullptr, *mel_lin = nullptr, *mel = nullptr, *logmag = nullptr, *energy = nullptr;
};

class Engine {
 public:
  explicit Engine(const tango_config_t& c);
  ~Engine();
  int init();

  int set_weight(const char* name, const float* dev, const int64_t* shape, int ndim);
  int finalize_weights();
  int denoise(const tango_denoise_args_t& a, hipStream_t s);
  struct Cond { const float* emb = nullptr; const uint8_t* mask = nullptr; int len = 0; const uint8_t* mask_host = nullptr; };
  int unet_forward(const float* sample, int64_t t, const Cond (&c)[3], float* out, int B2, hipStream_t s);
  int vae_decode(const float* lat, float* mel, int B, hipStream_t s);
  int vae_encode(const float* mel, float* moments, int B, hipStream_t s);
  int vocode(const float* mel, int16_t* wav, int B, int frames, int* n_samples, hipStream_t s);
  int vocoder_samples(int frames) const;
  int encode_text(const int64_t* ids, const uint8_t* mask, float* out, int B, int L, hipStream_t s);
  int mel_spectrogram(const float* wav, float* mel, float* logmag, float* energy, int B, int N, int* n_frames, hipStream_t s);
  int last_denoise_ms(float* total_ms, float* per_step_ms);
  int profile_unet(int B2, int L, std::string& report, hipStream_t s);
  int profile_vae(int B, std::string& report, hipStream_t s);
  int profile_vocoder(int B, int frames, std::string& report, hipStream_t s);
  void set_plan_budget(size_t bytes) { plan_budget = bytes; }
  void drop_plans() { const size_t b = plan_budget; plan_budget = 0; (void)make_room(1); plan_budget = b; }
  size_t plan_bytes_in_use() const { return plan_bytes; }
  int plan_count() const;

  tango_config_t cfg;
  int dt = DT_F32;
  size_t esz = 4;
  std::vector<Slot> slots;
  std::unordered_map<std::string, int> slot_index;
  bool finalized = false;
  float last_total_ms = 0.f, last_step_ms = 0.f;
  double last_step_gflop = 0.0;
  uint64_t coop_fallbacks = 0;

 private:
  friend struct Builder;
  std::vector<void*> owned;
  void* dmalloc(size_t bytes);
  void reg_slot(const std::string& name, std::vector<int64_t> shape, std::function<int(const float*, hipStream_t)> pack);
  void reg_vec(const std::string& name, int n, float** dst);
  void reg_norm(const std::string& p, int C, float eps, WNorm& w);
  void reg_mat(const std::string& wname, int N, int K, WMat& w, bool alloc, int row_off, std::vector<int64_t> shape, bool geglu = false);
  void reg_linear(const std::string& p, int N, int K, WMat& w, bool bias);
  void reg_conv3x3(const std::string& p, int Cout, int Cin, WMat& w);
  void reg_conv1x1(const std::string& p, int Cout, int Cin, WMat& w);
  void reg_conv1d(const std::string& p, int Cout, int Cin, int k, WMat& w);
  void reg_convt1d(const std::string& p, int Cin, int Cout, int k, int u, ConvTW& w);
  void reg_linear_f32(const std::string& p, int N, int K, WLinF32& w);
  void reg_res(const std::string& p, int cin, int cout, int temb, float eps, ResW& w, bool vae);
  void reg_xf(const std::string& p, int C, int heads, int cross, XfW& w);
  int fold_ln(WMat& w, const WNorm& ln);
  void build_unet_weights();
  void build_vae_weights();
  void build_vae_enc_weights();
  void reg_vae_attn(const std::string& p, int C, VaeAttnW& w);
  void build_voc_weights();
  void build_t5_weights();
  void build_stft_weights();

  WMat conv_in, conv_out;
  WNorm norm_out;
  WLinF32 time1, time2;
  struct DownBlock { std::vector<ResW> res; std::vector<XfW> xf, xf2, xf3; bool has_ds = false; WMat ds; };
  struct UpBlock { std::vector<ResW> res; std::vector<XfW> xf, xf2, xf3; bool has_us = false; WMat us; };
  std::vector<DownBlock> down;
  std::vector<UpBlock> up;
  ResW mid_res0, mid_res1;
  XfW mid_xf, mid_xf2, mid_xf3;
  std::vector<ResW*> all_res;
  std::vector<XfW*> all_xf;
  float* pqc_w = nullptr; float* pqc_b = nullptr;
  WMat vae_conv_in, vae_conv_out;
  ResW vae_mid1, vae_mid2;
  VaeAttnW vae_attn;
  struct VaeUp { std::vector<ResW> res; bool has_up = false; WMat up; };
  std::vector<VaeUp> vae_up;
  WNorm vae_norm_out;
  struct VaeDown { std::vector<ResW> res; bool has_down = false; WMat down; };
  std::vector<VaeDown> vae_down;
  WMat vae_enc_conv_in, vae_enc_conv_out;
  ResW vae_enc_mid1, vae_enc_mid2;
  VaeAttnW vae_enc_attn;
  WNorm vae_enc_norm_out;
  float* qc_w = nullptr; float* qc_b = nullptr;
  WMat voc_pre, voc_post;
  std::vector<ConvTW> voc_ups;
  std::vector<VocResW> voc_res;

  WMat stft_basis, stft_mel;
  std::map<std::pair<int, int>, std::unique_ptr<StftPlan>> stft_plans;
  int get_stft_plan(int B, int N, StftPlan** out);

  float* t5_embed = nullptr;
  float* t5_rel_table = nullptr;
  std::vector<T5LayerW> t5_layers;
  WNorm t5_final_ln;
  std::map<std::pair<int, int>, std::unique_ptr<T5Plan>> t5_plans;
  int get_t5_plan(int B, int L, T5Plan** out);
  int build_t5(T5Plan& P, Arena& A, bool record);

  int* d_step = nullptr;
  unsigned* d_sync = nullptr;
  SchedParams* d_sched = nullptr;
  int64_t* d_ts = nullptr;
  float* d_coef = nullptr;
  float* d_bcoef = nullptr;
  float* d_ring = nullptr;
  int ring_batch = 0;
  float* d_sin = nullptr;
  float* d_t1 = nullptr;
  float* d_temb = nullptr;
  std::vector<int64_t> temb_ts;
  int max_steps = 1000;
  std::map<std::array<int, 6>, std::unique_ptr<UNetPlan>> unet_plans;
  std::map<int, std::unique_ptr<VaePlan>> vae_plans;
  std::map<int, std::unique_ptr<VaePlan>> vae_enc_plans;
  std::map<std::pair<int, int>, std::unique_ptr<VaePlan>> voc_plans;
  hipEvent_t ev0 = nullptr, ev1 = nullptr;
  hipStream_t cap_stream = nullptr;
  hipStream_t cap_stream2 = nullptr, aux_stream = nullptr;
  hipEvent_t ev_fork = nullptr, ev_join = nullptr, ev_fork_e = nullptr, ev_join_e = nullptr;
  unsigned* d_sync2 = nullptr;
  int last_steps = 0;

  struct HostSlot { void* buf = nullptr; hipEvent_t ev = nullptr; bool pending = false; };
  static constexpr int kHostSlots = 8;
  static constexpr size_t kHostSlotBytes = 64 << 10;
// ... 33 lines not shown
```

tango_amd/csrc/engine.hip:

```cpp
#include "engine.h"
#include "tuning.h"

#include <algorithm>
#include <cmath>
#include <cstdio>
#include <cstring>

namespace tango {

static thread_local std::string g_err;
void set_error(const std::string& msg) { g_err = msg; }
const char* last_error() { return g_err.c_str(); }

struct GOpt {
  const float* bias2 = nullptr;
  int bias2_stride = 0;
  const TView* residual = nullptr;
  int a_act = ACT_NONE;
  float a_slope = 0.f;
  int e_act = ACT_NONE;
  float e_slope = 0.f;
  int epi = EPI_NONE;
  bool out_f32 = false;
  bool use_bias = true;
// ... 54 lines not shown
    }
    char buf[160];
    snprintf(buf, sizeof buf, "%s M=%d N=%d K=%d%s%s", what, p.M, p.N, p.K, p.batch > 1 ? " batched" : "", sk > 1 ? " splitK" : "");
    push([p, d](hipStream_t s) { return launch_gemm(d, p, s); }, buf, 2.0 * p.M * (double)p.N * p.K * p.batch);
  }


  void linear(const TView& x, int64_t rows, const WMat& w, const TView& out, const GOpt& o = GOpt()) {
    GemmParams p;
    p.A = x.p; p.lda = x.ld; p.W = w.W; p.Kp = w.Kp;
    p.bias = o.use_bias ? w.b : nullptr;
    p.M = (int)rows; p.N = w.N; p.K = w.K; p.Cin = w.K;
    p.mode = GATHER_1D; p.rows_pb = (int)rows; p.Lin = (int)rows; p.Lout = (int)rows; p.taps = 1;
    p.out = out.p; p.ldo = out.ld; p.out_f32 = o.out_f32;
    if (o.residual) { p.R = o.residual->p; p.ldr = o.residual->ld; }
    p.a_act = o.a_act; p.a_slope = o.a_slope; p.e_act = o.e_act; p.e_slope = o.e_slope; p.epi = o.epi; p.glu_tanh = o.glu_tanh;
    p.bias2 = o.bias2; p.bias2_stride = o.bias2_stride; p.step_ptr = o.bias2 ? E.d_step : nullptr;
    if (o.vt) { p.epi = EPI_VT; p.vt = o.vt; p.vt_n0 = o.vt_n0; p.vt_S = o.vt_S; p.vt_ld = o.vt_ld; p.vt_perm = o.vt_perm; }
    if (o.ln) {
      GemmParams q = p;
      q.W = w.Wln; q.bias = w.bln; q.ln_fold = 1; q.ln_eps = o.ln->eps; q.wsum = w.wsum;
      if (w.Wln && gemm_ln_fold_ok(dt, q)) {
        const int rq = gemm_route(dt, q);
        gemm(q, rq == ROUTE_WIDE ? "linear+ln(wide)" : rq == ROUTE_DUO ? "linear+ln(duo)" : "linear+ln(stream)");
        return;
      }
      if (w.Wln && p.epi == EPI_GEGLU && !tuning().no_ln_xstats) {
        const size_t m = A.mark();
        float* st = alloc_f32((size_t)rows * 2);
        GemmParams q2 = q;
        q2.row_stats = st;
        if (gemm_wide_ok(dt, q2) && gemm_route(dt, q2) == ROUTE_WIDE) {
          const int d = dt;
          const void* xp = x.p; const int64_t ldx = x.ld; const int r = (int)rows, c = o.ln->C; const float eps = o.ln->eps;
          push([=](hipStream_t s) { return launch_ln_stats(d, xp, ldx, st, r, c, eps, s); }, "ln_stats C=" + std::to_string(c));
          gemm(q2, "linear+ln(xstats)");
          A.release(m);
          return;
        }
        A.release(m);
      }
      const size_t m = A.mark();
      TView t = alloc(rows, o.ln->C);
      layernorm(x, rows, *o.ln, t);
      p.A = t.p; p.lda = t.ld;
      gemm(p, "linear");
      A.release(m);
      return;
    }
    if (o.rowvec && o.rowvec_rows > 0 && !tuning().no_rowvec_fuse) {
      GemmParams q = p;
      q.rowvec = o.rowvec; q.rowvec_rows = o.rowvec_rows; q.rowvec_per = o.rowvec_per;
      q.out_lo = o.out_lo ? o.out_lo->p : p.out; q.ldo_lo = o.out_lo ? o.out_lo->ld : p.ldo;
      if (gemm_rowvec_ok(dt, q)) {
        p = q;
        if (o.rowvec_done) *o.rowvec_done = true;
      }
    }
    const int route = gemm_pick_splitk(dt, p) > 1 ? ROUTE_TILE : gemm_route(dt, p);
    gemm(p, route == ROUTE_STREAM ? "linear(stream)" : route == ROUTE_WIDE ? "linear(wide)" : route == ROUTE_DUO ? "linear(duo)" : "linear");
  }

  void conv3x3(const TView& x, int B, int H, int W, int Hin, int Win, int stride, int ups, const WMat& w, const TView& out,
               const GOpt& o = GOpt()) {
    if (w.im2col) {
      const size_t m = A.mark();
      TView col = alloc((int64_t)B * H * W, (int)w.Kp);
      const int d = dt;
      const void* src = x.p; const int64_t ld = x.ld; void* dst = col.p; const int64_t Kp = w.Kp; const int Cs = w.Cin;
      push([=](hipStream_t s) { return launch_im2col3x3(d, src, ld, dst, Kp, B, H, W, Cs, s); });
      WMat lw = w; lw.K = (int)w.Kp; lw.im2col = false;
      linear(col, (int64_t)B * H * W, lw, out, o);
      A.release(m);
      return;
    }
    GemmParams p;
    p.A = x.p; p.lda = x.ld; p.W = w.W; p.Kp = w.Kp; p.bias = o.use_bias ? w.b : nullptr;
    p.M = B * H * W; p.N = w.N; p.K = w.K; p.Cin = w.Cin;
    p.mode = GATHER_2D; p.H = H; p.Wd = W; p.Hin = Hin; p.Win = Win; p.stride = stride; p.ups = ups; p.pad = o.pad;
    p.out = out.p; p.ldo = out.ld; p.out_f32 = o.out_f32;
    if (o.residual) { p.R = o.residual->p; p.ldr = o.residual->ld; }
    p.a_act = o.a_act; p.a_slope = o.a_slope; p.e_act = o.e_act; p.e_slope = o.e_slope; p.epi = o.epi;
    p.bias2 = o.bias2; p.bias2_stride = o.bias2_stride; p.step_ptr = o.bias2 ? E.d_step : nullptr;
    gemm(p, stride == 2 ? "conv3x3s2" : (ups ? "conv3x3up" : "conv3x3"));
  }

  bool linear_gn_fold(const TView& x, int B, int rows, const WNorm& gn, int groups, const WMat& w, const TView& out) {
    GroupNormParams gp;
    gp.x = x.p; gp.ldx = x.ld; gp.y = nullptr; gp.ldy = 0; gp.gamma = gn.g; gp.beta = gn.b;
    gp.B = B; gp.rows = rows; gp.C = gn.C; gp.groups = groups; gp.eps = gn.eps; gp.act = ACT_NONE;
    gp.sync = nullptr;
    if (w.K != gn.C || !gn_fold_ok(dt, gp, w.N)) return false;
    GemmParams p;
    p.A = x.p; p.lda = x.ld; p.Kp = w.Kp; p.bias = nullptr;
    p.M = B * rows; p.N = w.N; p.K = w.K; p.Cin = w.K;
    p.mode = GATHER_1D; p.rows_pb = p.M; p.Lin = p.M; p.Lout = p.M; p.taps = 1;
    p.out = out.p; p.ldo = out.ld;
    p.wb_rows = rows; p.wb_stride = (int64_t)w.N * w.Kp;
    p.rowvec_rows = p.M; p.rowvec_per = rows; p.out_lo = out.p; p.ldo_lo = out.ld;
    const size_t m = A.mark();
    void* Wf = A.alloc((size_t)B * w.N * w.Kp * esz);
    float* bf = alloc_f32((size_t)B * w.N);
    const size_t nf = groupnorm_ws_floats(B, rows, gn.C, groups);
    float* ws = alloc_f32(nf);
    gp.partial = ws; gp.scale_shift = nullptr;
    p.W = Wf; p.rowvec = bf;
    if (gemm_pick_splitk(dt, p) > 1 || !gemm_rowvec_ok(dt, p)) { A.release(m); return false; }
    const int d = dt;
    const void* Wsrc = w.W; const int64_t Kp = w.Kp; const float* bsrc = w.b; const int N = w.N;
    push([=](hipStream_t s) { return launch_gn_stats_fold(d, gp, Wsrc, Kp, bsrc, N, Wf, bf, s); },
         "groupnorm(fold) C=" + std::to_string(gn.C) + " rows=" + std::to_string(rows));
    gemm(p, gemm_route(dt, p) == ROUTE_DUO ? "linear(duo)" : "linear(wide)");
    A.release(m);
    return true;
  }

  bool gn_proj_stat(const TView& x, int B, int rows, const XfW& w, int groups, const TView& out) {
    if (!tuning().gn_proj_stat || !w.proj_in.Wln || (int64_t)B * rows < tuning().qkv_min_rows) return false;
    GroupNormParams gp;
    gp.x = x.p; gp.ldx = x.ld; gp.y = nullptr; gp.ldy = 0; gp.gamma = w.gn.g; gp.beta = w.gn.b;
    gp.B = B; gp.rows = rows; gp.C = w.C; gp.groups = groups; gp.eps = w.gn.eps; gp.act = ACT_NONE; gp.sync = nullptr;
    QKVParams q;
    q.x = x.p; q.ldx = x.ld; q.w = w.proj_in.Wln; q.ldw = w.proj_in.Kp; q.b = w.proj_in.bln; q.out = out.p; q.ldo = out.ld;
    q.M = B * rows; q.N = w.proj_in.N; q.K = w.C; q.n_rm = q.N; q.ln = 2; q.groups = groups; q.rows_ps = rows; q.eps = w.gn.eps;
    q.gstats = (const float*)(uintptr_t)16;
    if (!gn_stats_mr_ok(dt, gp) || !qkv_stat_ok(dt, q)) return false;
    const size_t m = A.mark();
    float* ws = alloc_f32(groupnorm_ws_floats(B, rows, w.C, groups));
    float* mr = alloc_f32((size_t)B * groups * 2);
    gp.partial = ws; gp.scale_shift = nullptr;
    q.gstats = mr;
    const int d = dt;
    push([=](hipStream_t s) { return launch_gn_stats_mr(d, gp, mr, s); }, "groupnorm(stats) C=" + std::to_string(w.C) + " rows=" + std::to_string(rows));
    char buf[96];
    snprintf(buf, sizeof buf, "linear+gn(stat) M=%d N=%d K=%d", q.M, q.N, q.K);
    push([q, d](hipStream_t s) { return launch_qkv_stat(d, q, s); }, buf, 2.0 * q.M * (double)q.N * q.K);
    A.release(m);
    return true;
  }

  bool qkv_stat(const TView& x, int64_t rows, const XfW& w, const TView& qk, void* vt, int HW, int vt_perm) {
    if (!tuning().qkv_stat || !w.qkv.Wln || rows < tuning().qkv_min_rows) return false;
    QKVParams q;
    q.x = x.p; q.ldx = x.ld; q.w = w.qkv.Wln; q.ldw = w.qkv.Kp; q.b = w.qkv.bln; q.out = qk.p; q.ldo = qk.ld; q.vt = vt; q.vt_ld = HW; q.vt_S = HW;
    q.M = (int)rows; q.N = 3 * w.C; q.K = w.C; q.n_rm = 2 * w.C; q.ln = 1; q.eps = w.ln1.eps; q.vt_perm = vt_perm;
    if (!qkv_stat_ok(dt, q)) return false;
    const int d = dt;
    char buf[96];
    snprintf(buf, sizeof buf, "qkv_stat M=%d N=%d K=%d", q.M, q.N, q.K);
    push([q, d](hipStream_t s) { return launch_qkv_stat(d, q, s); }, buf, 2.0 * rows * (double)q.N * q.K);
    return true;
  }

  bool ff_fused(const TView& x, int64_t rows, const XfW& w, const TView& out) {
    if (!tuning().ff_fused || !w.ff1.Wln || rows < tuning().ff_min_rows) return false;
    FFParams f;
    f.x = x.p; f.ldx = x.ld; f.w1 = w.ff1.Wln; f.ld1 = w.ff1.Kp; f.b1 = w.ff1.bln; f.w2 = w.ff2.W; f.ld2 = w.ff2.Kp; f.b2 = w.ff2.b;
    f.out = out.p; f.ldo = out.ld; f.M = (int)rows; f.C = w.C; f.H = 4 * w.C; f.eps = w.ln3.eps;
    if (!ff_fused_ok(dt, f)) return false;
    const int d = dt;
    char buf[96];
    snprintf(buf, sizeof buf, "ff_fused M=%d C=%d", f.M, f.C);
    push([f, d](hipStream_t s) { return launch_ff_fused(d, f, s); }, buf, 2.0 * rows * (double)(8 * w.C) * w.C + 2.0 * rows * (double)(4 * w.C) * w.C);
    return true;
  }

// ... 307 lines not shown
  }
  for (auto& c : P.child) if (c) { free_unet_plan(*c); c.reset(); }
  release_slab(&P.slab, P.meta);
}

int Engine::make_room(size_t need) {
  while (plan_bytes + need > plan_budget)
    if (!evict_lru()) break;
  return 0;
}

void Engine::release_slab(char** slab, PlanMeta& m) {
  if (*slab) (void)hipFree(*slab);
  *slab = nullptr;
  plan_bytes -= m.bytes < plan_bytes ? m.bytes : plan_bytes;
  m.bytes = 0;
}

int Engine::alloc_slab(char** slab, size_t bytes, PlanMeta& m, bool zero) {
  TANGO_TRY(make_room(bytes));
  for (;;) {
    const hipError_t e = hipMalloc((void**)slab, bytes);
    if (e == hipSuccess) break;
    (void)hipGetLastError();
    if (e != hipErrorOutOfMemory || !evict_lru())
      TANGO_FAIL(std::string("hipMalloc of a ") + std::to_string(bytes >> 20) + "-MiB plan workspace failed: " + hipGetErrorString(e));
  }
  if (zero && hipMemset(*slab, 0, bytes) != hipSuccess) { (void)hipGetLastError(); (void)hipFree(*slab); *slab = nullptr; TANGO_FAIL("hipMemset of a plan workspace failed"); }
  m.bytes = bytes;
  plan_bytes += bytes;
  touch(m);
  return 0;
}

void Engine::reg_slot(const std::string& name, std::vector<int64_t> shape, std::function<int(const float*, hipStream_t)> pack) {
  Slot s;
  s.name = name;
  s.shape = std::move(shape);
  s.pack = std::move(pack);
  slot_index[name] = (int)slots.size();
  slots.push_back(std::move(s));
}

void Engine::reg_vec(const std::string& name, int n, float** dst) {
  *dst = (float*)dmalloc((size_t)n * 4);
  float* d = *dst;
  reg_slot(name, {n}, [d, n](const float* src, hipStream_t s) {
    TANGO_HIP(hipMemcpyAsync(d, src, (size_t)n * 4, hipMemcpyDeviceToDevice, s));
    return 0;
  });
}

void Engine::reg_norm(const std::string& p, int C, float eps, WNorm& w) {
  w.C = C;
  w.eps = eps;
  reg_vec(p + ".weight", C, &w.g);
  reg_vec(p + ".bias", C, &w.b);
}

void Engine::reg_mat(const std::string& wname, int N, int K, WMat& w, bool alloc, int row_off, std::vector<int64_t> shape, bool geglu) {
  if (alloc) {
    w.K = K; w.Cin = K; w.taps = 1; w.Kp = K;
    w.W = dmalloc((size_t)w.N * w.Kp * esz);
  }
  void* W = w.W;
  const int64_t Kp = w.Kp;
  const int d = dt;
  const int64_t ro = geglu ? -1 : row_off;
  reg_slot(wname, std::move(shape), [=](const float* src, hipStream_t s) { return launch_pack(d, src, W, N, 1, K, K, 0, 1, Kp, ro, s); });
}

void Engine::reg_linear(const std::string& p, int N, int K, WMat& w, bool bias) {
  w.N = N;
  reg_mat(p + ".weight", N, K, w, true, 0, {N, K});
  if (bias) reg_vec(p + ".bias", N, &w.b);
}

void Engine::reg_conv1x1(const std::string& p, int Cout, int Cin, WMat& w) {
  w.N = Cout;
  reg_mat(p + ".weight", Cout, Cin, w, true, 0, {Cout, Cin, 1, 1});
  reg_vec(p + ".bias", Cout, &w.b);
}

void Engine::reg_conv3x3(const std::string& p, int Cout, int Cin, WMat& w) {
  w.N = Cout;
  w.im2col = ((Cin * esz) % 64) != 0;
  if (w.im2col) {
    w.Kp = ((9 * Cin + 31) / 32) * 32;
    w.K = 9 * Cin; w.Cin = Cin; w.taps = 9;
  } else {
    w.Kp = 9 * Cin; w.K = 9 * Cin; w.Cin = Cin; w.taps = 9;
  }
  w.W = dmalloc((size_t)Cout * w.Kp * esz);
  void* W = w.W;
  const int64_t Kp = w.Kp;
  const int d = dt;
  reg_slot(p + ".weight", {Cout, Cin, 3, 3},
           [=](const float* src, hipStream_t s) { return launch_pack(d, src, W, Cout, 9, Cin, (int64_t)Cin * 9, 1, 9, Kp, 0, s); });
  reg_vec(p + ".bias", Cout, &w.b);
}

void Engine::reg_conv1d(const std::string& p, int Cout, int Cin, int k, WMat& w) {
  w.N = Cout; w.K = k * Cin; w.Cin = Cin; w.taps = k; w.Kp = (int64_t)k * Cin;
  w.W = dmalloc((size_t)Cout * w.Kp * esz);
  void* W = w.W;
  const int64_t Kp = w.Kp;
  const int d = dt;
  reg_slot(p + ".weight", {Cout, Cin, k},
           [=](const float* src, hipStream_t s) { return launch_pack(d, src, W, Cout, k, Cin, (int64_t)Cin * k, 1, k, Kp, 0, s); });
  reg_vec(p + ".bias", Cout, &w.b);
}

void Engine::reg_convt1d(const std::string& p, int Cin, int Cout, int k, int u, ConvTW& w) {
  w.cin = Cin; w.cout = Cout; w.k = k; w.u = u; w.pad = (k - u) / 2;
  w.phase.resize(u);
  std::vector<void*> Ws(u);
  std::vector<int> Ts(u);
  for (int r = 0; r < u; ++r) {
    const int T = (k - r + u - 1) / u;
    WMat& m = w.phase[r];
    m.N = Cout; m.taps = T; m.Cin = Cin; m.K = T * Cin; m.Kp = (int64_t)T * Cin;
    m.W = dmalloc((size_t)Cout * m.Kp * esz);
    Ws[r] = m.W; Ts[r] = T;
  }
  const int d = dt;
  reg_slot(p + ".weight", {Cin, Cout, k}, [=](const float* src, hipStream_t s) {
    for (int r = 0; r < u; ++r)
      TANGO_TRY(launch_pack(d, src + r, Ws[r], Cout, Ts[r], Cin, k, u, (int64_t)Cout * k, (int64_t)Ts[r] * Cin, 0, s));
    return 0;
  });
  reg_vec(p + ".bias", Cout, &w.b);
  for (int r = 0; r < u; ++r) w.phase[r].b = w.b;
}

void Engine::reg_linear_f32(const std::string& p, int N, int K, WLinF32& w) {
  w.N = N; w.K = K;
  w.W = (float*)dmalloc((size_t)N * K * 4);
  float* W = w.W;
  reg_slot(p + ".weight", {N, K}, [=](const float* src, hipStream_t s) {
    TANGO_HIP(hipMemcpyAsync(W, src, (size_t)N * K * 4, hipMemcpyDeviceToDevice, s));
    return 0;
  });
  reg_vec(p + ".bias", N, &w.b);
}

void Engine::reg_res(const std::string& p, int cin, int cout, int temb, float eps, ResW& w, bool vae) {
  w.cin = cin; w.cout = cout;
  reg_norm(p + ".norm1", cin, eps, w.n1);
  reg_conv3x3(p + ".conv1", cout, cin, w.c1);
  if (temb > 0) {
    w.has_temb = true;
    reg_linear_f32(p + ".time_emb_proj", cout, temb, w.temb);
    w.temb_table = (float*)dmalloc((size_t)max_steps * cout * 4);
  }
  reg_norm(p + ".norm2", cout, eps, w.n2);
  reg_conv3x3(p + ".conv2", cout, cout, w.c2);
  if (cin != cout) {
    w.has_sc = true;
    reg_conv1x1(p + (vae ? ".nin_shortcut" : ".conv_shortcut"), cout, cin, w.sc);
  }
}

void Engine::reg_xf(const std::string& p, int C, int heads, int cross, XfW& w) {
  w.C = C; w.heads = heads;
  reg_norm(p + ".norm", C, 1e-6f, w.gn);
  reg_linear(p + ".proj_in", C, C, w.proj_in, true);
  const std::string b = p + ".transformer_blocks.0";
  w.qkv.N = 3 * C; w.qkv.K = C; w.qkv.Cin = C; w.qkv.Kp = C; w.qkv.taps = 1;
  w.qkv.W = dmalloc((size_t)3 * C * C * esz);
  reg_mat(b + ".attn1.to_q.weight", C, C, w.qkv, false, 0, {C, C});
  reg_mat(b + ".attn1.to_k.weight", C, C, w.qkv, false, C, {C, C});
  reg_mat(b + ".attn1.to_v.weight", C, C, w.qkv, false, 2 * C, {C, C});
  reg_linear(b + ".attn1.to_out.0", C, C, w.o1, true);
  w.ff1.N = 8 * C;
  reg_mat(b + ".ff.net.0.proj.weight", 8 * C, C, w.ff1, true, 0, {8 * C, C}, true);
  {
    w.ff1.b = (float*)dmalloc((size_t)8 * C * 4);
    float* d = w.ff1.b;
    const int n = 8 * C;
    reg_slot(b + ".ff.net.0.proj.bias", {n}, [d, n](const float* src, hipStream_t s) { return launch_permute_geglu_bias(src, d, n, s); });
  }
// ... 3 lines not shown
  w.kv2.W = dmalloc((size_t)2 * C * cross * esz);
  reg_mat(b + ".attn2.to_k.weight", C, cross, w.kv2, false, 0, {C, cross});
  reg_mat(b + ".attn2.to_v.weight", C, cross, w.kv2, false, C, {C, cross});
  reg_linear(b + ".attn2.to_out.0", C, C, w.o2, true);
  reg_norm(b + ".norm1", C, 1e-5f, w.ln1);
  reg_norm(b + ".norm2", C, 1e-5f, w.ln2);
  reg_norm(b + ".norm3", C, 1e-5f, w.ln3);
  reg_linear(p + ".proj_out", C, C, w.proj_out, true);
}

void Engine::build_unet_weights() {
  const int nl = cfg.unet_levels;
  const int* ch = cfg.unet_channels;
  const int temb = ch[0] * 4;
  const int cross = cfg.unet_cross_dim;
  const int lpb = cfg.unet_layers_per_block;
  const float eps = cfg.unet_eps;
  const std::string P = "unet.";
  reg_conv3x3(P + "conv_in", ch[0], cfg.unet_in_channels, conv_in);
  reg_linear_f32(P + "time_embedding.linear_1", temb, ch[0], time1);
  reg_linear_f32(P + "time_embedding.linear_2", temb, temb, time2);
  down.resize(nl);
  int cprev = ch[0];
  for (int i = 0; i < nl; ++i) {
    DownBlock& d = down[i];
    d.res.resize(lpb);
    if (cfg.unet_cross_attn[i]) {
      d.xf.resize(lpb);
      if (cfg.unet_music) { d.xf2.resize(lpb); d.xf3.resize(lpb); }
    }
    for (int j = 0; j < lpb; ++j) {
      const std::string bp = P + "down_blocks." + std::to_string(i);
      reg_res(bp + ".resnets." + std::to_string(j), j == 0 ? cprev : ch[i], ch[i], temb, eps, d.res[j], false);
      if (cfg.unet_cross_attn[i]) {
        reg_xf(bp + ".attentions." + std::to_string(j), ch[i], cfg.unet_heads[i], cross, d.xf[j]);
        if (cfg.unet_music) {
          reg_xf(bp + ".attentions2." + std::to_string(j), ch[i], cfg.unet_heads[i], cross, d.xf2[j]); d.xf2[j].cond = 1;
          reg_xf(bp + ".attentions3." + std::to_string(j), ch[i], cfg.unet_heads[i], cross, d.xf3[j]); d.xf3[j].cond = 2;
        }
      }
    }
    if (i != nl - 1) {
      d.has_ds = true;
      reg_conv3x3(P + "down_blocks." + std::to_string(i) + ".downsamplers.0.conv", ch[i], ch[i], d.ds);
    }
    cprev = ch[i];
  }
  const int cm = ch[nl - 1];
  reg_res(P + "mid_block.resnets.0", cm, cm, temb, eps, mid_res0, false);
  reg_xf(P + "mid_block.attentions.0", cm, cfg.unet_heads[nl - 1], cross, mid_xf);
  if (cfg.unet_music) {
    reg_xf(P + "mid_block.attentions2.0", cm, cfg.unet_heads[nl - 1], cross, mid_xf2); mid_xf2.cond = 1;
    reg_xf(P + "mid_block.attentions3.0", cm, cfg.unet_heads[nl - 1], cross, mid_xf3); mid_xf3.cond = 2;
  }
  reg_res(P + "mid_block.resnets.1", cm, cm, temb, eps, mid_res1, false);
  up.resize(nl);
  int prev_out = ch[nl - 1];
  for (int i = 0; i < nl; ++i) {
    const int lvl = nl - 1 - i;
    const int outc = ch[lvl];
    const int inc = ch[std::max(lvl - 1, 0)];
    UpBlock& u = up[i];
    const bool xa = cfg.unet_cross_attn[lvl] != 0;
    u.res.resize(lpb + 1);
    if (xa) {
      u.xf.resize(lpb + 1);
      if (cfg.unet_music) { u.xf2.resize(lpb + 1); u.xf3.resize(lpb + 1); }
    }
    const std::string bp = P + "up_blocks." + std::to_string(i);
    for (int j = 0; j <= lpb; ++j) {
      const int skip = (j == lpb) ? inc : outc;
      const int rin = (j == 0) ? prev_out : outc;
      reg_res(bp + ".resnets." + std::to_string(j), rin + skip, outc, temb, eps, u.res[j], false);
      if (xa) {
        reg_xf(bp + ".attentions." + std::to_string(j), outc, cfg.unet_heads[lvl], cross, u.xf[j]);
        if (cfg.unet_music) {
          reg_xf(bp + ".attentions2." + std::to_string(j), outc, cfg.unet_heads[lvl], cross, u.xf2[j]); u.xf2[j].cond = 1;
          reg_xf(bp + ".attentions3." + std::to_string(j), outc, cfg.unet_heads[lvl], cross, u.xf3[j]); u.xf3[j].cond = 2;
        }
      }
    }
    if (i != nl - 1) {
      u.has_us = true;
      reg_conv3x3(bp + ".upsamplers.0.conv", outc, outc, u.us);
    }
    prev_out = outc;
  }
  reg_norm(P + "conv_norm_out", ch[0], eps, norm_out);
  reg_conv3x3(P + "conv_out", cfg.unet_out_channels, ch[0], conv_out);
  auto push_xfs = [&](std::vector<XfW>& a, std::vector<XfW>& b, std::vector<XfW>& c) {
    for (auto& x : a) all_xf.push_back(&x);
    for (auto& x : b) all_xf.push_back(&x);
    for (auto& x : c) all_xf.push_back(&x);
  };
  for (auto& d : down) { for (auto& r : d.res) all_res.push_back(&r); push_xfs(d.xf, d.xf2, d.xf3); }
  all_res.push_back(&mid_res0); all_res.push_back(&mid_res1); all_xf.push_back(&mid_xf);
  if (cfg.unet_music) { all_xf.push_back(&mid_xf2); all_xf.push_back(&mid_xf3); }
  for (auto& u : up) { for (auto& r : u.res) all_res.push_back(&r); push_xfs(u.xf, u.xf2, u.xf3); }
}

void Engine::build_vae_weights() {
  const int nl = cfg.vae_levels;
  const int ch = cfg.vae_ch;
  const int zc = cfg.vae_z_channels, ed = cfg.vae_embed_dim;
  pqc_w = (float*)dmalloc((size_t)zc * ed * 4);
  {
    float* d = pqc_w;
    const size_t n = (size_t)zc * ed;
    reg_slot("post_quant_conv.weight", {zc, ed, 1, 1}, [d, n](const float* src, hipStream_t s) {
      TANGO_HIP(hipMemcpyAsync(d, src, n * 4, hipMemcpyDeviceToDevice, s));
      return 0;
    });
  }
  reg_vec("post_quant_conv.bias", zc, &pqc_b);
  const std::string D = "decoder.";
  int bi = ch * cfg.vae_ch_mult[nl - 1];
  reg_conv3x3(D + "conv_in", bi, zc, vae_conv_in);
  reg_res(D + "mid.block_1", bi, bi, 0, 1e-6f, vae_mid1, true);
  reg_vae_attn(D + "mid.attn_1", bi, vae_attn);
  reg_res(D + "mid.block_2", bi, bi, 0, 1e-6f, vae_mid2, true);
  vae_up.resize(nl);
  for (int lvl = nl - 1; lvl >= 0; --lvl) {
    const int bo = ch * cfg.vae_ch_mult[lvl];
    VaeUp& u = vae_up[lvl];
    u.res.resize(cfg.vae_num_res_blocks + 1);
    for (int b = 0; b <= cfg.vae_num_res_blocks; ++b) {
      reg_res(D + "up." + std::to_string(lvl) + ".block." + std::to_string(b), bi, bo, 0, 1e-6f, u.res[b], true);
      bi = bo;
    }
    if (lvl != 0) {
      u.has_up = true;
      reg_conv3x3(D + "up." + std::to_string(lvl) + ".upsample.conv", bi, bi, u.up);
    }
  }
  reg_norm(D + "norm_out", bi, 1e-6f, vae_norm_out);
  reg_conv3x3(D + "conv_out", cfg.vae_out_ch, bi, vae_conv_out);
}

void Engine::reg_vae_attn(const std::string& a, int bi, VaeAttnW& w) {
  reg_norm(a + ".norm", bi, 1e-6f, w.gn);
  w.qk.N = 2 * bi; w.qk.K = bi; w.qk.Cin = bi; w.qk.Kp = bi; w.qk.taps = 1;
  w.qk.W = dmalloc((size_t)2 * bi * bi * esz);
  w.qk.b = (float*)dmalloc((size_t)2 * bi * 4);
  reg_mat(a + ".q.weight", bi, bi, w.qk, false, 0, {bi, bi, 1, 1});
  reg_mat(a + ".k.weight", bi, bi, w.qk, false, bi, {bi, bi, 1, 1});
  {
    float* b0 = w.qk.b;
    float* b1 = w.qk.b + bi;
    const size_t n = (size_t)bi * 4;
    reg_slot(a + ".q.bias", {bi}, [b0, n](const float* src, hipStream_t s) { TANGO_HIP(hipMemcpyAsync(b0, src, n, hipMemcpyDeviceToDevice, s)); return 0; });
    reg_slot(a + ".k.bias", {bi}, [b1, n](const float* src, hipStream_t s) { TANGO_HIP(hipMemcpyAsync(b1, src, n, hipMemcpyDeviceToDevice, s)); return 0; });
  }
  reg_conv1x1(a + ".v", bi, bi, w.v);
  reg_conv1x1(a + ".proj_out", bi, bi, w.proj);
}

void Engine::build_vae_enc_weights() {
  const int nl = cfg.vae_levels, ch = cfg.vae_ch, zc = cfg.vae_z_channels, ed = cfg.vae_embed_dim;
  const int cin = cfg.vae_in_channels > 0 ? cfg.vae_in_channels : 1;
  const std::string E = "encoder.";
  reg_conv3x3(E + "conv_in", ch, cin, vae_enc_conv_in);
  vae_down.resize(nl);
  int bi = ch;
  for (int lvl = 0; lvl < nl; ++lvl) {
    const int bo = ch * cfg.vae_ch_mult[lvl];
    VaeDown& d = vae_down[lvl];
    d.res.resize(cfg.vae_num_res_blocks);
// ... 1254 lines not shown
```

tango_amd/csrc/gemm.hip:

```cpp
#include <cstdlib>

#include <map>
#include <mutex>
#include <utility>

#include "common.h"
#include "gemm_device.h"
#include "tuning.h"

namespace tango {

int ensure_dyn_lds(const void* kfn, int bytes) {
  static std::mutex mu;
  static std::map<std::pair<const void*, int>, int> opted;
  int dev = 0;
  TANGO_HIP(hipGetDevice(&dev));
  std::lock_guard<std::mutex> lock(mu);
  int& have = opted[std::make_pair(kfn, dev)];
  if (bytes > have) {
    TANGO_HIP(hipFuncSetAttribute(kfn, hipFuncAttributeMaxDynamicSharedMemorySize, bytes));
    have = bytes;
  }
  return 0;
}
// ... 275 lines not shown
                      p.Lin >= p.M;
  if (linear) return launch_tile<T, BKB, MODE_LINEAR>(p, s);
  return launch_tile<T, BKB, MODE_CONV1D>(p, s);
}

template <typename T>
static int launch_t(const GemmParams& p, hipStream_t s) {
  const int cb = p.Cin * (int)sizeof(T);
  if (p.M <= 0 || p.N <= 0) return 0;
  if (p.K % p.Cin != 0) TANGO_FAIL("gemm: K must be taps*Cin");
  if (p.a_act != ACT_NONE && p.a_act != ACT_LRELU && p.a_act != ACT_SILU) TANGO_FAIL("gemm: the operand prologue implements leaky-ReLU and SiLU only");
  if ((p.lda * (int64_t)sizeof(T)) % 16 != 0 || (p.Kp * (int64_t)sizeof(T)) % 16 != 0) TANGO_FAIL("gemm: lda/Kp must be 16-byte multiples");
  if (cb % 128 == 0) return launch_mode<T, 128>(p, s);
  if (cb % 64 == 0) return launch_mode<T, 64>(p, s);
  TANGO_FAIL("gemm: Cin*sizeof(T) must be a multiple of 64 bytes");
}

static unsigned char* g_zero_page = nullptr;

int gemm_init() {
  if (!g_zero_page) {
    TANGO_HIP(hipMalloc((void**)&g_zero_page, 4096));
    TANGO_HIP(hipMemset(g_zero_page, 0, 4096));
  }
  return 0;
}

int gemm_pick_splitk(int dtype, const GemmParams& p) {
  if (p.batch != 1 || p.epi != EPI_NONE || p.bias_rows || p.out_scale != 1.f || (p.N & 3) || (p.ldo & 3) || (p.R && (p.ldr & 3)))
    return 1;
  if (p.mode == GATHER_1D && !(p.taps == 1 && p.rows_pb == p.M && p.in_mul == 1 && p.in_off == 0 && p.out_mul == 1 && p.out_off == 0))
    return 1;
  if (gemm_duo_ok(dtype, p) || linear_stream_ok(dtype, p)) return 1;
  if (small_tile_linear(p, dtype == DT_F32 ? 4 : 2)) return 1;
  if (p.N <= 32 && conv_halo_ok(dtype, p)) return 1;
  {
    const int sw = conv_wide_pick_splitk(dtype, p);
    if (sw > 1) return sw;
  }
  const int esz = dtype == DT_F32 ? 4 : 2;
  const int bk = ((p.Cin * esz) % 128 == 0) ? 128 / esz : 64 / esz;
  const int nk = p.K / bk;
  const int bn = (p.N % 160 == 0) ? 160 : (p.N >= 96 ? 128 : (p.N > 32 ? 64 : 32));
  const int bm = p.N > 32 ? 128 : 256;
  const int tiles = ((p.M + bm - 1) / bm) * ((p.N + bn - 1) / bn);
  if (tiles >= 400) return 1;
  int s = (512 + tiles / 2) / tiles;
  if (s > nk / 3) s = nk / 3;
  if (s > 32) s = 32;
  return s < 2 ? 1 : s;
}

int gemm_route(int dtype, const GemmParams& p) {
  if (gemm_duo_ok(dtype, p)) return ROUTE_DUO;
  if (!p.ln_fold && gemm_wide_ok(dtype, p)) {
    return ROUTE_WIDE;
  }
  if (p.ln_fold && gemm_wide_ok(dtype, p)) return ROUTE_WIDE;
  if (linear_stream_ok(dtype, p)) return ROUTE_STREAM;
  if (p.ln_fold) return ROUTE_NONE;
  if (conv_wide_ok(dtype, p)) return ROUTE_CONV_WIDE;
  if (conv_halo_ok(dtype, p)) return ROUTE_CONV_HALO;
  if (gemm_wide_ok(dtype, p)) return ROUTE_WIDE;
  if (gemm_dma_ok(dtype, p)) return ROUTE_DMA;
  return ROUTE_TILE;
}

bool gemm_rowvec_ok(int dtype, const GemmParams& p) {
  if (p.epi != EPI_NONE || p.splitk > 1 || gemm_pick_splitk(dtype, p) > 1) return false;
  if (p.rowvec_rows % 64 != 0 || p.rowvec_per % 64 != 0 || p.rowvec_rows > p.M) return false;
  if (p.out_lo && (p.ldo_lo % 8 != 0 || ((uintptr_t)p.out_lo & 15))) return false;
  if ((uintptr_t)p.rowvec & 15) return false;
  const int r = gemm_route(dtype, p);
  return r == ROUTE_WIDE || r == ROUTE_DUO;
}

int launch_gemm(int dtype, const GemmParams& p, hipStream_t s) {
  if (p.rowvec && !gemm_rowvec_ok(dtype, p)) TANGO_FAIL("gemm: rowvec is only implemented by the 256 x 320 / 256 x 160 GEMM epilogues");
  const int route = gemm_route(dtype, p);
  if (p.epi == EPI_VT && p.vt_perm && (p.vt_S % 32 != 0 || dtype == DT_F32)) TANGO_FAIL("gemm: vt_perm permutes whole blocks of 32 tokens of a 16-bit V^T (vt_S % 32 == 0)");
  if (p.wb_rows && route != ROUTE_WIDE && route != ROUTE_DUO) TANGO_FAIL("gemm: per-sample weights are implemented by the 256 x 320 / 256 x 160 GEMMs only");
  if (p.glu_tanh && dtype != DT_F32 && route != ROUTE_WIDE && route != ROUTE_DUO)
    TANGO_FAIL("gemm: the tanh-GELU gate (T5 gated-gelu) is implemented by the fp32 kernels and the 256 x 320 / 256 x 160 GEMMs only");
  switch (route) {
    case ROUTE_WIDE: return launch_gemm_wide(dtype, p, s);
    case ROUTE_DUO: return launch_gemm_duo(dtype, p, s);
    case ROUTE_STREAM: return launch_linear_stream(dtype, p, s);
    case ROUTE_CONV_WIDE: return launch_conv_wide(dtype, p, g_zero_page, s);
    case ROUTE_CONV_HALO: return launch_conv_halo(dtype, p, g_zero_page, s);
    case ROUTE_DMA: return launch_gemm_dma(dtype, p, g_zero_page, s);
    case ROUTE_NONE: TANGO_FAIL("gemm: ln_fold is only implemented by the streaming linear and the 256 x 320 GEMM kernels");
    default: break;
  }
  switch (dtype) {
    case DT_F32: return launch_t<float>(p, s);
    case DT_F16: return launch_t<f16>(p, s);
    case DT_BF16: return launch_t<bf16>(p, s);
  }
  TANGO_FAIL("gemm: bad dtype");
}

}
```

tango_amd/csrc/gemm_wide_device.h:

```cpp
#pragma once
#include "common.h"
#include "gemm_device.h"

namespace tango {

constexpr int WIDE_STAGE_BYTES = 11520;

template <bool LN>
__device__ __forceinline__ f32x4 wide_col_value(const f32x4 av, const float mean, const float rstd, const float alpha, const float* cst) {
  const f32x4 cbv = *(const f32x4*)cst;
  f32x4 v;
  if (LN) {
    const f32x4 cwv = *(const f32x4*)(cst + 160);
#pragma unroll
    for (int r = 0; r < 4; ++r) {
      float t;
      asm("v_fma_f32 %0, -%1, %2, %3" : "=v"(t) : "v"(mean), "v"(cwv[r]), "v"(av[r]));
      v[r] = rstd * t + cbv[r];
    }
  } else {
    v = av * alpha + cbv;
  }
  return v;
}

template <typename T, bool GEGLU, bool RES, bool LN>
__device__ __forceinline__ void wide_epilogue(const GemmParams& p, f32x4 (&acc)[10][4], const float (&mean)[4], const float (&rstd)[4],
                                              const int m_base, const int n_base, const int lane, unsigned char* stage) {
  constexpr int TN = 10, NIT = 5;
  constexpr int OC = GEGLU ? 80 : 160;
  constexpr int PITCH = OC * 4 + 16;
  constexpr int PPR = OC / 8;
  constexpr int RPP = GEGLU ? 32 : 16;
  constexpr int NPASS = 64 / RPP;
  const int l15 = lane & 15, g4 = (lane >> 4) * 4;
  const float* bias2 = p.bias2 ? p.bias2 + (int64_t)(p.step_ptr ? *p.step_ptr : 0) * p.bias2_stride : nullptr;
  float* const cst = (float*)(stage + WIDE_STAGE_BYTES);
  const bool lo = !GEGLU && p.rowvec != nullptr && (int64_t)m_base < p.rowvec_rows;
  if (lane < 40) {
    f32x4 bv = p.bias ? *(const f32x4*)(p.bias + n_base + lane * 4) : f32x4{0.f, 0.f, 0.f, 0.f};
    if (bias2) bv += *(const f32x4*)(bias2 + n_base + lane * 4);
    if (lo) bv += *(const f32x4*)(p.rowvec + (int64_t)(m_base / p.rowvec_per) * p.N + n_base + lane * 4);
    *(f32x4*)(cst + lane * 4) = bv;
    if (LN) *(f32x4*)(cst + 160 + lane * 4) = *(const f32x4*)(p.wsum + n_base + lane * 4);
  }
  __builtin_amdgcn_wave_barrier();
  const int ocol0 = GEGLU ? (n_base >> 1) : n_base;
  const T* Rb = (const T*)p.R;
  T* Ob = lo ? (T*)p.out_lo : (T*)p.out;
  const int64_t ldo = lo ? p.ldo_lo : p.ldo;
  int prow[NIT], pcol[NIT];
#pragma unroll
  for (int it = 0; it < NIT; ++it) {
    const int idx = lane + it * 64;
    prow[it] = idx / PPR;
    pcol[it] = (idx - prow[it] * PPR) * 8;
  }
  u32x4 rv[2][NIT];
  auto fetch_res = [&](const int ps, u32x4 (&dst)[NIT]) {
#pragma unroll
    for (int it = 0; it < NIT; ++it)
      dst[it] = *(const u32x4*)(Rb + (int64_t)(m_base + ps * RPP + prow[it]) * p.ldr + ocol0 + pcol[it]);
  };
  if (RES) fetch_res(0, rv[0]);
#pragma unroll
  for (int ps = 0; ps < NPASS; ++ps) {
#pragma unroll
    for (int bb = 0; bb < RPP / 16; ++bb) {
      const int b = ps * (RPP / 16) + bb;
#pragma unroll
      for (int a = 0; a < TN; a += GEGLU ? 2 : 1) {
        f32x4 v = wide_col_value<LN>(acc[a][b], mean[b], rstd[b], p.alpha, cst + a * 16 + g4);
        if (GEGLU) {
          const f32x4 gv = wide_col_value<LN>(acc[a + 1][b], mean[b], rstd[b], p.alpha, cst + (a + 1) * 16 + g4);
          const float gt[4] = {gv[0], gv[1], gv[2], gv[3]};
          glu_gate4<T>(v, gt, p.glu_tanh);
        }
        *(f32x4*)(stage + (bb * 16 + l15) * PITCH + ((GEGLU ? (a >> 1) : a) * 16 + g4) * 4) = v;
      }
    }
    if (RES && ps + 1 < NPASS) fetch_res(ps + 1, rv[(ps + 1) & 1]);
    __builtin_amdgcn_wave_barrier();
    if (RES) {
      if (ps == 0) { if (NPASS > 1) wait_vmcnt_lit<NIT>(); else wait_vmcnt_lit<0>(); }
      else if (ps + 1 < NPASS) wait_vmcnt_lit<2 * NIT>();
      else wait_vmcnt_lit<NIT>();
    }
#pragma unroll
    for (int it = 0; it < NIT; ++it) {
      const f32x4 lo = *(const f32x4*)(stage + prow[it] * PITCH + pcol[it] * 4);
      const f32x4 hi = *(const f32x4*)(stage + prow[it] * PITCH + pcol[it] * 4 + 16);
      float f[8] = {lo[0], lo[1], lo[2], lo[3], hi[0], hi[1], hi[2], hi[3]};
      if (RES) {
        T r8[8];
        __builtin_memcpy(r8, &rv[ps & 1][it], 16);
#pragma unroll
        for (int e = 0; e < 8; ++e) f[e] += to_f(r8[e]);
      }
      if (p.out_scale != 1.f) {
#pragma unroll
        for (int e = 0; e < 8; ++e) f[e] *= p.out_scale;
      }
      T tv[8];
#pragma unroll
      for (int e = 0; e < 8; ++e) tv[e] = from_f<T>(f[e]);
      u32x4 o;
      __builtin_memcpy(&o, tv, 16);
      *(u32x4*)(Ob + (int64_t)(m_base + ps * RPP + prow[it]) * ldo + ocol0 + pcol[it]) = o;
    }
    __builtin_amdgcn_wave_barrier();
  }
}


template <typename T, bool LN>
__device__ __forceinline__ void wide_epilogue_vt(const GemmParams& p, f32x4 (&acc)[10][4], const float (&mean)[4], const float (&rstd)[4],
                                                 const int m_base, const int n_base, const int lane, unsigned char* stage) {
  constexpr int TN = 10, TM = 4, CPITCH = 64 * 2 + 16;
  const int l15 = lane & 15, g4 = (lane >> 4) * 4;
  float* const cst = (float*)(stage + WIDE_STAGE_BYTES);
  if (lane < 40) {
    *(f32x4*)(cst + lane * 4) = p.bias ? *(const f32x4*)(p.bias + n_base + lane * 4) : f32x4{0.f, 0.f, 0.f, 0.f};
    if (LN) *(f32x4*)(cst + 160 + lane * 4) = *(const f32x4*)(p.wsum + n_base + lane * 4);
  }
  __builtin_amdgcn_wave_barrier();
  const int bb = m_base / p.vt_S, s0 = m_base - bb * p.vt_S;
  T* const vbase = (T*)p.vt + ((int64_t)bb * (p.N - p.vt_n0) + (n_base - p.vt_n0)) * p.vt_ld + s0;
  int tpos[TM];
#pragma unroll
  for (int b = 0; b < TM; ++b) tpos[b] = p.vt_perm ? vt_perm_pos(b * 16 + l15) : b * 16 + l15;
#pragma unroll
  for (int ps = 0; ps < 2; ++ps) {
#pragma unroll
    for (int al = 0; al < TN / 2; ++al) {
      const int a = ps * (TN / 2) + al;
#pragma unroll
      for (int b = 0; b < TM; ++b) {
        const f32x4 v = wide_col_value<LN>(acc[a][b], mean[b], rstd[b], p.alpha, cst + a * 16 + g4);
#pragma unroll
        for (int r = 0; r < 4; ++r) *(T*)(stage + (al * 16 + g4 + r) * CPITCH + tpos[b] * 2) = from_f<T>(v[r]);
      }
    }
    __builtin_amdgcn_wave_barrier();
#pragma unroll
    for (int it = 0; it < 10; ++it) {
      const int idx = lane + it * 64, col = idx >> 3, pc = idx & 7;
      const u32x4 o = *(const u32x4*)(stage + col * CPITCH + pc * 16);
      *(u32x4*)(vbase + (int64_t)(ps * 80 + col) * p.vt_ld + pc * 8) = o;
    }
    __builtin_amdgcn_wave_barrier();
  }
}


__device__ __forceinline__ void wide_epilogue_raw(const GemmParams& p, f32x4 (&acc)[10][4], const int split, const int m_base, const int n_base,
                                                  const int lane, unsigned char* stage) {
  constexpr int PITCH = 160 * 4 + 16;
  const int l15 = lane & 15, g4 = (lane >> 4) * 4;
  float* const wsb = p.ws + ((int64_t)split * p.M + m_base) * p.N + n_base;
#pragma unroll
  for (int b = 0; b < 4; ++b) {
#pragma unroll
    for (int a = 0; a < 10; ++a) *(f32x4*)(stage + l15 * PITCH + (a * 16 + g4) * 4) = acc[a][b];
    __builtin_amdgcn_wave_barrier();
#pragma unroll
    for (int it = 0; it < 10; ++it) {
      const int idx = lane + it * 64, row = idx / 40, pc = idx - row * 40;
      *(f32x4*)(wsb + (int64_t)(b * 16 + row) * p.N + pc * 4) = *(const f32x4*)(stage + row * PITCH + pc * 16);
    }
    __builtin_amdgcn_wave_barrier();
  }
}

}
```

tango_amd/csrc/ops_abi.hip:

```cpp
#include <string>
#include <vector>

#include "../../include/tango_engine.h"
#include "common.h"
#include "tuning.h"

namespace tango {

struct Scratch {
  std::vector<void*> ptrs;
  ~Scratch() { for (void* p : ptrs) (void)hipFree(p); }
  void* get(size_t bytes) {
    void* p = nullptr;
    if (hipMalloc(&p, bytes ? bytes : 256) != hipSuccess) return nullptr;
    ptrs.push_back(p);
    return p;
  }
};

template <typename T>
__global__ void to_f32_kernel(const T* __restrict__ src, int64_t ld, float* __restrict__ dst, int64_t rows, int C) {
  const int64_t i = (int64_t)blockIdx.x * 256 + threadIdx.x;
  if (i >= rows * C) return;
  const int64_t r = i / C;
  dst[i] = to_f(src[r * ld + (i - r * C)]);
}
static int to_f32(int dt, const void* src, int64_t ld, float* dst, int64_t rows, int C, hipStream_t s) {
  const unsigned nb = (unsigned)((rows * C + 255) / 256);
  switch (dt) {
    case DT_F32: hipLaunchKernelGGL((to_f32_kernel<float>), dim3(nb), dim3(256), 0, s, (const float*)src, ld, dst, rows, C); break;
    case DT_F16: hipLaunchKernelGGL((to_f32_kernel<f16>), dim3(nb), dim3(256), 0, s, (const f16*)src, ld, dst, rows, C); break;
    case DT_BF16: hipLaunchKernelGGL((to_f32_kernel<bf16>), dim3(nb), dim3(256), 0, s, (const bf16*)src, ld, dst, rows, C); break;
    default: TANGO_FAIL("to_f32: bad dtype");
  }
  TANGO_HIP(hipGetLastError());
  return 0;
}

template <typename T>
__global__ void transpose_v_kernel(const T* __restrict__ v, T* __restrict__ vt, int B, int S, int C, int64_t ldvt) {
  const int64_t i = (int64_t)blockIdx.x * 256 + threadIdx.x;
  if (i >= (int64_t)B * S * C) return;
  const int c = (int)(i % C);
  const int64_t bs = i / C;
  const int s = (int)(bs % S), b = (int)(bs / S);
  vt[((int64_t)b * C + c) * ldvt + s] = v[i];
}
static int transpose_v(int dt, const void* v, void* vt, int B, int S, int C, int64_t ldvt, hipStream_t s) {
  const unsigned nb = (unsigned)(((int64_t)B * S * C + 255) / 256);
  switch (dt) {
    case DT_F32: hipLaunchKernelGGL((transpose_v_kernel<float>), dim3(nb), dim3(256), 0, s, (const float*)v, (float*)vt, B, S, C, ldvt); break;
    case DT_F16: hipLaunchKernelGGL((transpose_v_kernel<f16>), dim3(nb), dim3(256), 0, s, (const f16*)v, (f16*)vt, B, S, C, ldvt); break;
    case DT_BF16: hipLaunchKernelGGL((transpose_v_kernel<bf16>), dim3(nb), dim3(256), 0, s, (const bf16*)v, (bf16*)vt, B, S, C, ldvt); break;
    default: TANGO_FAIL("transpose_v: bad dtype");
  }
  TANGO_HIP(hipGetLastError());
  return 0;
}

}

using namespace tango;

static int run_gemm(int dt, GemmParams& p, Scratch& sc, hipStream_t s) {
  TANGO_TRY(gemm_init());
  const int sk = gemm_pick_splitk(dt, p);
  if (sk > 1) {
    p.splitk = sk;
    p.ws = (float*)sc.get((size_t)sk * p.M * p.N * 4);
    if (!p.ws) TANGO_FAIL("run_gemm: alloc");
  }
  return launch_gemm(dt, p, s);
}

extern "C" {

int tango_op_conv2d(int dt, const float* x, const float* w, const float* bias, float* out, int B, int Cin, int H, int W, int Cout,
                    int stride, int upsample, void* stream) {
  hipStream_t s = (hipStream_t)stream;
  const size_t esz = dtype_size(dt);
  Scratch sc;
  const int Hc = H << upsample, Wc = W << upsample;
  const int Ho = stride == 2 ? (Hc + 2 - 3) / 2 + 1 : Hc, Wo = stride == 2 ? (Wc + 2 - 3) / 2 + 1 : Wc;
  const bool im2col = ((Cin * esz) % 64) != 0;
  const int cpad = im2col ? ((Cin + 7) / 8) * 8 : Cin;
  void* xt = sc.get((size_t)B * H * W * cpad * esz);
  void* ot = sc.get((size_t)B * Ho * Wo * Cout * esz);
  if (!xt || !ot) TANGO_FAIL("op_conv2d: alloc");
  TANGO_HIP(hipMemsetAsync(xt, 0, (size_t)B * H * W * cpad * esz, s));
  TANGO_TRY(launch_nchw_to_nhwc(dt, x, xt, cpad, B, Cin, H * W, 1, 1.0f, s));
  GemmParams p;
  p.bias = bias; p.N = Cout; p.out = ot; p.ldo = Cout;
  if (im2col) {
    if (stride != 1 || upsample) TANGO_FAIL("op_conv2d: small-Cin path supports stride 1 only");
    const int64_t Kp = ((9 * Cin + 31) / 32) * 32;
    void* wt = sc.get((size_t)Cout * Kp * esz);
    void* col = sc.get((size_t)B * H * W * Kp * esz);
    if (!wt || !col) TANGO_FAIL("op_conv2d: alloc");
    TANGO_TRY(launch_pack(dt, w, wt, Cout, 9, Cin, (int64_t)Cin * 9, 1, 9, Kp, 0, s));
    TANGO_TRY(launch_im2col3x3(dt, xt, cpad, col, Kp, B, H, W, Cin, s));
    p.A = col; p.lda = Kp; p.W = wt; p.Kp = Kp; p.M = B * H * W; p.K = (int)Kp; p.Cin = (int)Kp;
    p.mode = GATHER_1D; p.rows_pb = p.M; p.Lin = p.M; p.Lout = p.M;
  } else {
    const int64_t Kp = 9 * Cin;
    void* wt = sc.get((size_t)Cout * Kp * esz);
    if (!wt) TANGO_FAIL("op_conv2d: alloc");
    TANGO_TRY(launch_pack(dt, w, wt, Cout, 9, Cin, (int64_t)Cin * 9, 1, 9, Kp, 0, s));
    p.A = xt; p.lda = cpad; p.W = wt; p.Kp = Kp; p.M = B * Ho * Wo; p.K = 9 * Cin; p.Cin = Cin;
    p.mode = GATHER_2D; p.H = Ho; p.Wd = Wo; p.Hin = H; p.Win = W; p.stride = stride; p.ups = upsample;
  }
  TANGO_TRY(run_gemm(dt, p, sc, s));
  TANGO_TRY(launch_nhwc_to_nchw_f32(dt, ot, Cout, out, B, Cout, Ho * Wo, s));
  TANGO_HIP(hipStreamSynchronize(s));
  return 0;
}

int tango_op_linear(int dt, const float* x, const float* w, const float* bias, const float* residual, float* out, int M, int N,
                    int K, int a_act, int e_act, int geglu, void* stream) {
  hipStream_t s = (hipStream_t)stream;
  const size_t esz = dtype_size(dt);
  Scratch sc;
  const int No = geglu ? N / 2 : N;
  void* xt = sc.get((size_t)M * K * esz);
  void* wt = sc.get((size_t)N * K * esz);
  void* ot = sc.get((size_t)M * No * esz);
  void* rt = residual ? sc.get((size_t)M * No * esz) : nullptr;
  float* bt = bias ? (float*)sc.get((size_t)N * 4) : nullptr;
  if (!xt || !wt || !ot) TANGO_FAIL("op_linear: alloc");
  TANGO_TRY(launch_cast_rows(dt, x, xt, K, M, K, s));
  TANGO_TRY(launch_pack(dt, w, wt, N, 1, K, K, 0, 1, K, geglu ? -1 : 0, s));
  if (residual) TANGO_TRY(launch_cast_rows(dt, residual, rt, No, M, No, s));
  if (bias) {
    if (geglu) TANGO_TRY(launch_permute_geglu_bias(bias, bt, N, s));
    else TANGO_HIP(hipMemcpyAsync(bt, bias, (size_t)N * 4, hipMemcpyDeviceToDevice, s));
  }
  GemmParams p;
  p.A = xt; p.lda = K; p.W = wt; p.Kp = K; p.bias = bt; p.M = M; p.N = N; p.K = K; p.Cin = K;
  p.mode = GATHER_1D; p.rows_pb = M; p.Lin = M; p.Lout = M;
  p.out = ot; p.ldo = No; p.R = rt; p.ldr = No; p.a_act = a_act; p.e_act = e_act; p.epi = geglu ? EPI_GEGLU : EPI_NONE;
  TANGO_TRY(run_gemm(dt, p, sc, s));
  TANGO_TRY(to_f32(dt, ot, No, out, M, No, s));
  TANGO_HIP(hipStreamSynchronize(s));
  return 0;
}

int tango_op_linear_ln(int dt, const float* x, const float* w, const float* bias, const float* gamma, const float* beta,
                       const float* residual, float* out, int M, int N, int K, int geglu, float eps, void* stream) {
  hipStream_t s = (hipStream_t)stream;
  const size_t esz = dtype_size(dt);
  Scratch sc;
  const int No = geglu ? N / 2 : N;
  void* xt = sc.get((size_t)M * K * esz);
  void* wt = sc.get((size_t)N * K * esz);
  void* wl = sc.get((size_t)N * K * esz);
  void* ot = sc.get((size_t)M * No * esz);
  void* rt = residual ? sc.get((size_t)M * No * esz) : nullptr;
  float* bt = (float*)sc.get((size_t)N * 4);
  float* bl = (float*)sc.get((size_t)N * 4);
  float* ws = (float*)sc.get((size_t)N * 4);
  if (!xt || !wt || !wl || !ot || !bt || !bl || !ws) TANGO_FAIL("op_linear_ln: alloc");
  TANGO_TRY(launch_cast_rows(dt, x, xt, K, M, K, s));
  TANGO_TRY(launch_pack(dt, w, wt, N, 1, K, K, 0, 1, K, geglu ? -1 : 0, s));
  if (residual) TANGO_TRY(launch_cast_rows(dt, residual, rt, No, M, No, s));
  if (bias) {
    if (geglu) TANGO_TRY(launch_permute_geglu_bias(bias, bt, N, s));
    else TANGO_HIP(hipMemcpyAsync(bt, bias, (size_t)N * 4, hipMemcpyDeviceToDevice, s));
  }
  TANGO_TRY(launch_fold_ln(dt, wt, K, gamma, beta, bias ? bt : nullptr, wl, bl, ws, N, K, s));
  GemmParams p;
  p.A = xt; p.lda = K; p.W = wl; p.Kp = K; p.bias = bl; p.M = M; p.N = N; p.K = K; p.Cin = K;
  p.mode = GATHER_1D; p.rows_pb = M; p.Lin = M; p.Lout = M;
  p.out = ot; p.ldo = No; p.R = rt; p.ldr = No; p.epi = geglu ? EPI_GEGLU : EPI_NONE;
  p.ln_fold = 1; p.ln_eps = eps; p.wsum = ws;
  TANGO_TRY(gemm_init());
  GemmParams px = p;
  px.row_stats = (float*)sc.get((size_t)M * 2 * 4);
  if (gemm_ln_fold_ok(dt, p)) {
    TANGO_TRY(launch_gemm(dt, p, s));
  } else if (geglu && !residual && px.row_stats && !tuning().no_ln_xstats && gemm_wide_ok(dt, px) && gemm_route(dt, px) == ROUTE_WIDE) {
    TANGO_TRY(launch_ln_stats(dt, xt, K, (float*)px.row_stats, M, K, eps, s));
    TANGO_TRY(launch_gemm(dt, px, s));
  } else {
    void* nt = sc.get((size_t)M * K * esz);
    if (!nt) TANGO_FAIL("op_linear_ln: alloc");
    TANGO_TRY(launch_layernorm(dt, xt, K, nt, K, gamma, beta, M, K, eps, s));
    p.A = nt; p.W = wt; p.bias = bias ? bt : nullptr; p.ln_fold = 0; p.wsum = nullptr;
    TANGO_TRY(launch_gemm(dt, p, s));
  }
  TANGO_TRY(to_f32(dt, ot, No, out, M, No, s));
  TANGO_HIP(hipStreamSynchronize(s));
  return 0;
}

const char* tango_debug_linear_route(int dt, int M, int N, int K, int geglu, int ln_fold, int residual, int vt) {
  static thread_local std::string out;
// ... 490 lines not shown
```

tango_amd/csrc/tuning.h:

```cpp
#pragma once
#include <cstdlib>

namespace tango {

struct Tuning {
  bool force_big_kernels;
  bool no_wide_conv;
  bool no_wide_gemm;
  bool no_halo_conv;
  bool no_dma_gemm;
  bool no_stream;
  bool no_small_tile;
  bool no_xattn_fused;
  bool no_single_key;
  int wide_prio;
  int wide_sched;
  bool no_stream_ln_geglu;
  bool no_rowvec_fuse;
  bool no_ln_xstats;
  bool no_gn_coop;
  bool gn_coop_all;
  bool gn_coop_force_fb;
  int graph_steps;
  int unet_chains;
  bool no_cfg_shared;
  bool stream_spec;
  int attn_qb2_min_wgs;
  bool no_halo_narrow;
  int gn_slab;
  int gn_small_mb;
  int wide_pers;
  bool attn_msum;
  int duo_maxk;
  int duo_min_tiles;
  int duo_mask;
  int duo_prio;
  int ff_fused;
  int ff_min_rows;
  int qkv_stat;
  int qkv_min_rows;
  int gn_proj_stat;
  bool gn_fold;
  int attn_kdma;
  int attn_vdma;
  int attn_defer;
  int attn_x8_qb;
  int conv_tall;
  int wide_pipe;
  int conv_pipe;
};

inline Tuning read_tuning() {
  auto on = [](const char* k) { const char* v = getenv(k); return v != nullptr && v[0] != '0'; };
  Tuning x;
  x.force_big_kernels = on("TANGO_FORCE_DMA_GEMM");
  x.no_wide_conv = on("TANGO_NO_WIDE_CONV");
  x.no_wide_gemm = on("TANGO_NO_WIDE_GEMM");
  x.no_halo_conv = on("TANGO_NO_HALO_CONV");
  x.no_dma_gemm = on("TANGO_NO_DMA_GEMM");
  x.no_stream = on("TANGO_NO_STREAM");
  x.no_small_tile = on("TANGO_NO_SMALL_TILE");
  x.no_xattn_fused = on("TANGO_NO_XATTN_FUSED");
  x.no_single_key = on("TANGO_NO_SINGLE_KEY");
  x.no_stream_ln_geglu = on("TANGO_NO_STREAM_LN_GEGLU");
  x.no_gn_coop = on("TANGO_NO_GN_COOP");
  x.no_ln_xstats = on("TANGO_NO_LN_XSTATS");
  x.no_rowvec_fuse = on("TANGO_NO_ROWVEC_FUSE");
  const char* ws = getenv("TANGO_WIDE_SCHED");
  x.wide_sched = (ws && ws[0] >= '0' && ws[0] <= '1') ? ws[0] - '0' : 1;
  auto num = [](const char* k, int dflt) { const char* v = getenv(k); return (v && v[0]) ? atoi(v) : dflt; };
  x.gn_coop_all = on("TANGO_GN_COOP_ALL");
  x.gn_coop_force_fb = on("TANGO_GN_COOP_FORCE_FALLBACK");
  x.graph_steps = num("TANGO_GRAPH_STEPS", 0);
  x.unet_chains = num("TANGO_UNET_CHAINS", 0);
  x.no_cfg_shared = on("TANGO_NO_CFG_SHARED");
  x.stream_spec = num("TANGO_STREAM_SPEC", 1) != 0;
  x.attn_qb2_min_wgs = num("TANGO_ATTN_QB2_MIN_WGS", 512);
  x.gn_small_mb = num("TANGO_GN_SMALL_MB", 8);
  x.gn_slab = num("TANGO_GN_SLAB", 1);
  x.no_halo_narrow = on("TANGO_NO_HALO_NARROW");
  x.wide_pers = num("TANGO_WIDE_PERS", 2);
  x.attn_msum = num("TANGO_ATTN_MSUM", 1) != 0;
  x.duo_maxk = num("TANGO_DUO_MAXK", -1);
  x.duo_min_tiles = num("TANGO_DUO_MIN_TILES", 384);
  x.duo_mask = num("TANGO_DUO_MASK", 7);
  x.duo_prio = num("TANGO_DUO_PRIO", 0);
  x.wide_pipe = num("TANGO_WIDE_PIPE", 0);
  x.conv_pipe = num("TANGO_CONV_PIPE", 2);
  x.conv_tall = num("TANGO_CONV_TALL", 0);
  x.attn_x8_qb = num("TANGO_ATTN_X8_QB", 2);
  x.attn_defer = num("TANGO_ATTN_DEFER", 0);
  x.attn_kdma = num("TANGO_ATTN_KDMA", 1);
  x.attn_vdma = num("TANGO_ATTN_VDMA", 2);
  x.gn_fold = on("TANGO_GN_FOLD");
  x.ff_fused = num("TANGO_FF_FUSED", 1);
  x.qkv_stat = num("TANGO_QKV_STAT", 1);
  x.gn_proj_stat = num("TANGO_GN_PROJ_STAT", 1);
  x.qkv_min_rows = num("TANGO_QKV_MIN_ROWS", 65536);
  x.ff_min_rows = num("TANGO_FF_MIN_ROWS", 32768);
  const char* wp = getenv("TANGO_WIDE_PRIO");
  x.wide_prio = (wp && wp[0] >= '0' && wp[0] <= '2') ? wp[0] - '0' : 0;
  return x;
}

inline Tuning& tuning_storage() {
  static Tuning t = read_tuning();
  return t;
}
inline const Tuning& tuning() { return tuning_storage(); }
inline void tuning_reload() { tuning_storage() = read_tuning(); }

}
```

tango_amd/weights.py:

```python
import zlib
from collections import OrderedDict
from typing import Dict, Iterator, Tuple

import torch

Shapes = "OrderedDict[str, Tuple[int, ...]]"


def _resnet(out, p, cin, cout, temb):
    out[p + ".norm1.weight"] = (cin,)
    out[p + ".norm1.bias"] = (cin,)
    out[p + ".conv1.weight"] = (cout, cin, 3, 3)
    out[p + ".conv1.bias"] = (cout,)
    out[p + ".time_emb_proj.weight"] = (cout, temb)
    out[p + ".time_emb_proj.bias"] = (cout,)
    out[p + ".norm2.weight"] = (cout,)
    out[p + ".norm2.bias"] = (cout,)
    out[p + ".conv2.weight"] = (cout, cout, 3, 3)
    out[p + ".conv2.bias"] = (cout,)
    if cin != cout:
        out[p + ".conv_shortcut.weight"] = (cout, cin, 1, 1)
        out[p + ".conv_shortcut.bias"] = (cout,)


# ... 181 lines not shown
            for m in range(len(cfg["resblock_dilation_sizes"][j])):
                out[f"{rp}.convs2.{m}.weight"] = (ch, ch, ks)
                out[f"{rp}.convs2.{m}.bias"] = (ch,)
    out[P + "conv_post.weight"] = (1, ch, 7)
    out[P + "conv_post.bias"] = (1,)
    return out


T5_CONFIG_LARGE = dict(vocab_size=32128, d_model=1024, d_kv=64, num_heads=16, d_ff=2816, num_layers=24,
                       relative_attention_num_buckets=32, relative_attention_max_distance=128, layer_norm_epsilon=1e-6)
T5_CONFIG_XL = dict(T5_CONFIG_LARGE, d_model=2048, num_heads=32, d_ff=5120)


def t5_encoder_param_shapes(cfg: dict, prefix: str = "text_encoder.") -> Shapes:
    d, inner, dff = cfg["d_model"], cfg["num_heads"] * cfg["d_kv"], cfg["d_ff"]
    out: Shapes = {}
    out[prefix + "shared.weight"] = (cfg["vocab_size"], d)
    out[prefix + "encoder.block.0.layer.0.SelfAttention.relative_attention_bias.weight"] = (cfg["relative_attention_num_buckets"], cfg["num_heads"])
    for i in range(cfg["num_layers"]):
        b = "%sencoder.block.%d" % (prefix, i)
        for n in ("q", "k", "v"):
            out["%s.layer.0.SelfAttention.%s.weight" % (b, n)] = (inner, d)
        out["%s.layer.0.SelfAttention.o.weight" % b] = (d, inner)
        out["%s.layer.0.layer_norm.weight" % b] = (d,)
        out["%s.layer.1.DenseReluDense.wi_0.weight" % b] = (dff, d)
        out["%s.layer.1.DenseReluDense.wi_1.weight" % b] = (dff, d)
        out["%s.layer.1.DenseReluDense.wo.weight" % b] = (d, dff)
        out["%s.layer.1.layer_norm.weight" % b] = (d,)
    out[prefix + "encoder.final_layer_norm.weight"] = (d,)
    return out


def stft_param_shapes(cfg: dict, prefix: str = "") -> Shapes:
    cutoff = cfg["filter_length"] // 2 + 1
    return {prefix + "stft_fn.forward_basis": (2 * cutoff, 1, cfg["filter_length"]), prefix + "mel_basis": (cfg["n_mel_channels"], cutoff)}


def t5_config_from_state_dict(sd, prefix: str = "text_encoder.") -> dict:
    d = sd[prefix + "shared.weight"].shape[1] if prefix + "shared.weight" in sd else sd[prefix + "encoder.embed_tokens.weight"].shape[1]
    vocab = (sd.get(prefix + "shared.weight", sd.get(prefix + "encoder.embed_tokens.weight"))).shape[0]
    rel = sd[prefix + "encoder.block.0.layer.0.SelfAttention.relative_attention_bias.weight"]
    inner = sd[prefix + "encoder.block.0.layer.0.SelfAttention.q.weight"].shape[0]
    layers = 1 + max(int(k[len(prefix):].split(".")[2]) for k in sd if k.startswith(prefix + "encoder.block."))
    if prefix + "encoder.block.0.layer.1.DenseReluDense.wi_0.weight" not in sd:
        raise ValueError("only gated-gelu T5 (v1.1 / FLAN-T5) encoders are supported")
    return dict(vocab_size=vocab, d_model=d, d_kv=inner // rel.shape[1], num_heads=rel.shape[1],
                d_ff=sd[prefix + "encoder.block.0.layer.1.DenseReluDense.wi_0.weight"].shape[0], num_layers=layers,
                relative_attention_num_buckets=rel.shape[0], relative_attention_max_distance=128, layer_norm_epsilon=1e-6)


def _is_norm(name: str) -> bool:
    leaf = name.rsplit(".", 2)[-2] if name.count(".") >= 1 else name
    return leaf.startswith("norm") or leaf in ("conv_norm_out", "norm_out")


def synth_tensor(name: str, shape: Tuple[int, ...], seed: int = 1234) -> torch.Tensor:
    g = torch.Generator()
    g.manual_seed((int(seed) * 1000003 + zlib.crc32(name.encode())) % (2 ** 63 - 1))
    if _is_norm(name):
        t = torch.randn(shape, generator=g)
        return (1.0 + 0.1 * t) if name.endswith(".weight") else 0.1 * t
    if len(shape) == 1:
        return (torch.rand(shape, generator=g) * 2 - 1) * 0.05
    if ".ups." in name and len(shape) == 3:
        fan_in = shape[0] * shape[2] / 4.0
    else:
        fan_in = 1
        for s in shape[1:]:
            fan_in *= s
    gain = 1.0
    if name.startswith("vocoder.") or ".vocoder." in name:
        gain = 3.0 ** 0.5
    b = gain / (fan_in ** 0.5)
    return (torch.rand(shape, generator=g) * 2 - 1) * b


def synth_state_dict(shapes: Shapes, seed: int = 1234) -> Dict[str, torch.Tensor]:
    return OrderedDict((k, synth_tensor(k, s, seed)) for k, s in shapes.items())


def iter_synth(shapes: Shapes, seed: int = 1234) -> Iterator[Tuple[str, torch.Tensor]]:
    for k, s in shapes.items():
        yield k, synth_tensor(k, s, seed)
```

Before: 32.18 audio-seconds/s.

## Fold nearest-upsample into 3x3 conv via four 2x2 phase kernels

Nearest-2x upsample followed by a 3x3 conv is rewritten as four sub-pixel phase convolutions with 2x2 kernels over the original-resolution input. Each phase kernel holds the summed original taps. This cuts the MACs and halo gather per output from 9 taps to 4, and the convolution reads the low-resolution input directly. The wide conv kernel gains a phase template that decodes the phase from the block index, uses 4 taps with an adjusted halo DMA schedule, and scatters its output rows into the interleaved high-resolution positions. The cost is extra phase-weight memory and packing at load time, plus a narrower set of problems the path accepts.

```diff
diff --git a/include/tango_engine.h b/include/tango_engine.h
--- a/include/tango_engine.h
+++ b/include/tango_engine.h
@@ -142,6 +142,9 @@
 
 int tango_op_conv2d(int dtype, const float* x, const float* w, const float* bias, float* out, int B, int Cin, int H, int W,
                     int Cout, int stride, int upsample, void* stream);
+int tango_op_conv2d_ups(int dtype, const float* x, const float* w, const float* bias, const float* bias2, float* out, int B, int Cin,
+                        int H, int W, int Cout, int phases, void* stream);
+int tango_op_pack_ups_phase(int dtype, const float* w, void* out, int Cout, int Cin, void* stream);
 int tango_op_linear(int dtype, const float* x, const float* w, const float* bias, const float* residual, float* out, int M,
                     int N, int K, int a_act, int e_act, int geglu, void* stream);
 int tango_op_linear_ln(int dtype, const float* x, const float* w, const float* bias, const float* gamma, const float* beta,
diff --git a/tango_amd/_lib.py b/tango_amd/_lib.py
--- a/tango_amd/_lib.py
+++ b/tango_amd/_lib.py
@@ -102,7 +102,7 @@
     "tango_engine_finalize_weights", "tango_engine_denoise", "tango_engine_unet_forward", "tango_engine_unet_forward_music",
     "tango_engine_vae_decode", "tango_engine_vae_encode", "tango_engine_vocode", "tango_engine_vocoder_samples", "tango_engine_encode_text",
     "tango_engine_mel_frames", "tango_engine_mel_spectrogram",
-    "tango_engine_last_denoise_ms", "tango_engine_last_step_gflop", "tango_engine_profile_unet", "tango_engine_profile_vae", "tango_engine_profile_vocoder", "tango_engine_set_plan_budget", "tango_engine_plan_stats", "tango_engine_drop_plans", "tango_op_conv2d", "tango_op_linear", "tango_op_linear_ln", "tango_op_ff_fused", "tango_op_qkv_stat", "tango_op_linear_qkv", "tango_op_linear_qkv_perm", "tango_op_conv1d",
+    "tango_engine_last_denoise_ms", "tango_engine_last_step_gflop", "tango_engine_profile_unet", "tango_engine_profile_vae", "tango_engine_profile_vocoder", "tango_engine_set_plan_budget", "tango_engine_plan_stats", "tango_engine_drop_plans", "tango_op_conv2d", "tango_op_conv2d_ups", "tango_op_pack_ups_phase", "tango_op_linear", "tango_op_linear_ln", "tango_op_ff_fused", "tango_op_qkv_stat", "tango_op_linear_qkv", "tango_op_linear_qkv_perm", "tango_op_conv1d",
     "tango_op_conv_transpose1d", "tango_op_groupnorm", "tango_op_layernorm", "tango_op_attention", "tango_op_attention_ex", "tango_op_xattn_block",
     "tango_op_sched_step", "tango_op_sched_multistep", "tango_op_philox_normal",
     "tango_op_sched_masked", "tango_op_philox_normal_blend",
@@ -153,6 +153,8 @@
     lib.tango_debug_linear_route.restype = C.c_char_p
     lib.tango_engine_plan_stats.argtypes = [vp, C.POINTER(C.c_uint64), C.POINTER(ci)]
     lib.tango_op_conv2d.argtypes = [ci, vp, vp, vp, vp, ci, ci, ci, ci, ci, ci, ci, vp]
+    lib.tango_op_conv2d_ups.argtypes = [ci, vp, vp, vp, vp, vp, ci, ci, ci, ci, ci, ci, vp]
+    lib.tango_op_pack_ups_phase.argtypes = [ci, vp, vp, ci, ci, vp]
     lib.tango_op_linear.argtypes = [ci, vp, vp, vp, vp, vp, ci, ci, ci, ci, ci, ci, vp]
     lib.tango_op_linear_ln.argtypes = [ci, vp, vp, vp, vp, vp, vp, vp, ci, ci, ci, ci, cf, vp]
     lib.tango_op_ff_fused.argtypes = [ci, vp, vp, vp, vp, vp, vp, vp, vp, ci, ci, ci, cf, ci, ci, vp, vp]
diff --git a/tango_amd/csrc/common.h b/tango_amd/csrc/common.h
--- a/tango_amd/csrc/common.h
+++ b/tango_amd/csrc/common.h
@@ -132,6 +132,7 @@
 struct GemmParams {
   const void* A = nullptr;
   const void* W = nullptr;
+  const void* Wph = nullptr;
   const float* bias = nullptr;
   const float* bias2 = nullptr;
   const int* step_ptr = nullptr;
@@ -195,6 +196,8 @@
 bool conv_wide_ok(int dtype, const GemmParams& p);
 int launch_conv_wide(int dtype, const GemmParams& p, const unsigned char* zero_page, hipStream_t s);
 int conv_wide_pick_splitk(int dtype, const GemmParams& p);
+bool conv_ups_phase_ok(int dtype, const GemmParams& p);
+int launch_pack_ups_phase(int dtype, const float* src, void* dst, int O, int I, hipStream_t s);
 int launch_splitk_reduce(int dtype, const GemmParams& p, hipStream_t s);
 bool gemm_dma_ok(int dtype, const GemmParams& p);
 int launch_gemm_dma(int dtype, const GemmParams& p, const unsigned char* zero_page, hipStream_t s);
diff --git a/tango_amd/csrc/conv_wide.hip b/tango_amd/csrc/conv_wide.hip
--- a/tango_amd/csrc/conv_wide.hip
+++ b/tango_amd/csrc/conv_wide.hip
@@ -14,7 +14,7 @@
 static constexpr int CW_HALO_MAX_TALL = 800;
 static constexpr int CW_NA_TALL = 7;
 
-template <typename T, bool RES, bool SK, int SCH, bool TALL>
+template <typename T, bool RES, bool SK, int SCH, bool TALL, bool PH = false>
 __global__ __launch_bounds__(512) void conv3x3_wide_kernel(const GemmParams p, const unsigned char* zero_page, const int SR, const int nseg,
                                                            const int abytes, const int prio) {
   constexpr int BM = TALL ? 512 : 256, BN = TALL ? 160 : 320, CB = 64, NST = 4;
@@ -24,6 +24,8 @@
   constexpr int WRG = BN / 16;
   constexpr int WRGW = (WRG + 7) / 8;
   constexpr int TM = 4, TN = 10;
+  constexpr int NTAP = PH ? 4 : 9;
+  static_assert(!PH || (SCH == 1 && !TALL && !SK && !RES), "phase form: the in-stream DMA schedule of the unsplit 256 x 320 tile");
   extern __shared__ __attribute__((aligned(16))) unsigned char dsm[];
   unsigned char* const As = dsm;
   unsigned char* const Ws = dsm + 2 * abytes;
@@ -34,6 +36,8 @@
     const int nblk = gridDim.x, q = nblk >> 3, r = nblk & 7, xcd = bid & 7, idx = bid >> 3;
     bid = (xcd < r ? xcd * (q + 1) : r * (q + 1) + (xcd - r) * q) + idx;
   }
+  const int phase = PH ? (bid & 3) : 0;
+  if (PH) bid >>= 2;
   const int m0 = (bid / NT) * BM, n0 = (bid % NT) * BN;
   const unsigned char* Ab = (const unsigned char*)p.A;
   const unsigned char* Wb = (const unsigned char*)p.W;
@@ -67,7 +71,7 @@
   const unsigned w_off0_init = (unsigned)(((int64_t)wrow_d * p.Kp) * (int64_t)sizeof(T) + ((slot ^ ((wrow_d >> 1) & 2)) * 16));
   aoff_lds[CW_NA * 512] = w_off0_init;
   const unsigned w_step = (unsigned)(128 * p.Kp * (int64_t)sizeof(T));
-  const unsigned char* const Wt = Wb + (int64_t)n0 * p.Kp * (int64_t)sizeof(T);
+  const unsigned char* const Wt = Wb + ((int64_t)phase * p.N + n0) * p.Kp * (int64_t)sizeof(T);
   const int my_w = wave < WRG - 8 * (WRGW - 1) ? WRGW : WRGW - 1;
 
   auto issue_a_off = [&](const int t, const int cc, const int buf, const unsigned off) {
@@ -133,7 +137,8 @@
     cc0 = (int)blockIdx.y * per;
     cc1 = cc1 < cc0 + per ? cc1 : cc0 + per;
   }
-  const int NI = (cc1 - cc0) * 9;
+  const int NI = (cc1 - cc0) * NTAP;
+  const int ph_off = PH ? (phase >> 1) * HW2 + (phase & 1) : 0;
 
   const int half = wave >> 2;
 #pragma unroll
@@ -148,25 +153,28 @@
   int st = 0, item = 0;
   int prev_h = 0;
   unsigned hoff = 0u;
+  unsigned hoff2 = 0u;
   unsigned w_off0 = w_off0_init;
   asm volatile("" : "+v"(w_off0));
   for (int cc = cc0; cc < cc1; ++cc) {
     const unsigned char* Ah = As + (cc & 1) * abytes;
     const bool more_c = cc + 1 < cc1;
 #pragma unroll 1
-    for (int tap = 0; tap < 9; ++tap, ++item) {
+    for (int tap = 0; tap < NTAP; ++tap, ++item) {
       const unsigned char* Wst = Ws + st * WST;
-      const int toff = (tap / 3) * HW2 + (tap % 3);
-      const bool iss_h = more_c && tap < CW_NA && tap * 8 + wave < HALO_RG;
+      const int toff = PH ? ph_off + (tap >> 1) * HW2 + (tap & 1) : (tap / 3) * HW2 + (tap % 3);
+      const bool iss_h = more_c && tap < (PH ? 3 : CW_NA) && tap * 8 + wave < HALO_RG;
+      const bool iss_h2 = PH && more_c && tap + 3 < CW_NA && (tap + 3) * 8 + wave < HALO_RG;
       const bool iss_w = item + 3 < NI;
       const int st3 = st == 0 ? 3 : st - 1;
       int koff3;
       {
         int t3 = tap + 3, c3 = cc;
-        if (t3 >= 9) { t3 -= 9; c3 = cc + 1; }
+        if (t3 >= NTAP) { t3 -= NTAP; c3 = cc + 1; }
         koff3 = (t3 * p.Cin + c3 * BK) * (int)sizeof(T);
       }
       if (SCH != 0) { if (iss_h) hoff = aoff_lds[tap * 512]; }
+      if (PH) { if (iss_h2) hoff2 = aoff_lds[(tap + 3) * 512]; }
       u32x4 wf[TN], xf[TM];
 #pragma unroll
       for (int a = 0; a < TN; ++a) wf[a] = *(const u32x4*)(Wst + wfoff + a * 16 * CB);
@@ -177,14 +185,14 @@
         const int h = h0 + hs;
         xf[b] = *(const u32x4*)(Ah + h * CB + ((kg ^ ((h >> 1) & 2)) << 4));
       }
-      if (item + 1 < NI) wait_n(prev_h + (item + 2 < NI ? my_w : 0));
-      prev_h = iss_h ? 1 : 0;
+      if (item + 1 < NI) wait_n((PH && tap == NTAP - 1 ? 0 : prev_h) + (item + 2 < NI ? my_w : 0));
+      prev_h = (iss_h ? 1 : 0) + (iss_h2 ? 1 : 0);
       pp_barrier();
       if (SCH == 0) {
         if (more_c && tap < CW_NA) issue_a(tap, cc + 1, (cc + 1) & 1);
         const int t3 = tap + 3;
-        if (t3 < 9) issue_w(t3, cc, st3);
-        else if (more_c) issue_w(t3 - 9, cc + 1, st3);
+        if (t3 < NTAP) issue_w(t3, cc, st3);
+        else if (more_c) issue_w(t3 - NTAP, cc + 1, st3);
       }
       if (prio == 0) __builtin_amdgcn_s_setprio(1);
 #pragma unroll
@@ -194,7 +202,10 @@
         if (SCH != 0 && (a & 1) == 0 && (a >> 1) <= WRGW) {
           const int sl = a >> 1;
           __builtin_amdgcn_sched_barrier(0);
-          if (sl == 0) { if (iss_h) issue_a_off(tap, cc + 1, (cc + 1) & 1, hoff); }
+          if (sl == 0) {
+            if (iss_h) issue_a_off(tap, cc + 1, (cc + 1) & 1, hoff);
+            if (PH) { if (iss_h2) issue_a_off(tap + 3, cc + 1, (cc + 1) & 1, hoff2); }
+          }
           else if (iss_w) issue_w_one(sl - 1, koff3, st3, w_off0);
           __builtin_amdgcn_sched_barrier(0);
         }
@@ -213,7 +224,7 @@
     return;
   }
   const float mean[TM] = {0.f, 0.f, 0.f, 0.f}, rstd[TM] = {1.f, 1.f, 1.f, 1.f};
-  wide_epilogue<T, false, RES, false>(p, acc, mean, rstd, m0 + wm * 64, n0 + wn * (TN * 16), lane, slice);
+  wide_epilogue<T, false, RES, false, PH>(p, acc, mean, rstd, m0 + wm * 64, n0 + wn * (TN * 16), lane, slice, phase);
 }
 
 template <int OFF> __device__ __forceinline__ void cwp_lds_read(u32x4& v, const unsigned base) {
@@ -553,6 +564,24 @@
   return tuning().force_big_kernels || tiles >= 224;
 }
 
+static GemmParams ups_phase_problem(const GemmParams& p) {
+  GemmParams q = p;
+  q.W = p.Wph; q.Wph = nullptr;
+  q.Kp = 4 * (int64_t)p.Cin; q.K = 4 * p.Cin;
+  q.M = p.M / 4; q.H = p.Hin; q.Wd = p.Win; q.ups = 0;
+  return q;
+}
+
+bool conv_ups_phase_ok(int dtype, const GemmParams& p) {
+  if (!tuning().ups_phases || p.ups != 1 || p.splitk > 1 || p.R || p.M % 1024 != 0) return false;
+  if (!conv_wide_ok(dtype, p)) return false;
+  GemmParams q = ups_phase_problem(p);
+  q.W = p.W;
+  if ((int64_t)4 * p.N * q.Kp * 2 >= (int64_t)0xFFFF0000) return false;
+  WideHaloGeom g;
+  return wide_halo_geom(q, g);
+}
+
 int conv_wide_pick_splitk(int dtype, const GemmParams& p) {
   GemmParams q = p;
   q.splitk = 1;
@@ -586,6 +615,24 @@
   return 0;
 }
 
+template <typename T>
+static int launch_conv_wide_phase(int dtype, const GemmParams& p, const unsigned char* zero_page, hipStream_t s) {
+  if (!conv_ups_phase_ok(dtype, p) || ((uintptr_t)p.Wph & 15)) TANGO_FAIL("conv_wide: phase weights given for a problem the phase form does not take");
+  const GemmParams q = ups_phase_problem(p);
+  WideHaloGeom g;
+  if (!wide_halo_geom(q, g)) TANGO_FAIL("conv_wide: unsupported geometry");
+  const int abytes = ((g.halo + 15) / 16) * 1024;
+  int lds = 2 * abytes + 4 * 320 * 64 + (CW_NA_WIDE + 1) * 512 * 4;
+  const int epi_lds = 8 * (WIDE_STAGE_BYTES + 1280);
+  if (lds < epi_lds) lds = epi_lds;
+  auto kfn = conv3x3_wide_kernel<T, false, false, 1, false, true>;
+  TANGO_TRY(ensure_dyn_lds(reinterpret_cast<const void*>(kfn), lds));
+  const int tiles = (q.M / 256) * (q.N / 320);
+  hipLaunchKernelGGL(kfn, dim3((unsigned)(4 * tiles)), dim3(512), lds, s, q, zero_page, g.SR, g.nseg, abytes, tuning().wide_prio);
+  TANGO_HIP(hipGetLastError());
+  return 0;
+}
+
 template <typename T, bool RES, bool SK>
 static int launch_conv_wide_pipe(const GemmParams& p, const unsigned char* zero_page, hipStream_t s) {
   WideHaloGeom g;
@@ -618,6 +665,7 @@
 
 int launch_conv_wide(int dtype, const GemmParams& p, const unsigned char* zero_page, hipStream_t s) {
   if (!zero_page) TANGO_FAIL("conv_wide: gemm_init() was not called (zero page for the LDS-DMA gather)");
+  if (p.Wph) return dtype == DT_F16 ? launch_conv_wide_phase<f16>(dtype, p, zero_page, s) : launch_conv_wide_phase<bf16>(dtype, p, zero_page, s);
   switch (dtype) {
     case DT_F16:
       if (p.splitk > 1) return launch_conv_wide_cfg<f16, false, true>(p, zero_page, s);
diff --git a/tango_amd/csrc/elementwise.hip b/tango_amd/csrc/elementwise.hip
--- a/tango_amd/csrc/elementwise.hip
+++ b/tango_amd/csrc/elementwise.hip
@@ -478,6 +478,35 @@
   return 0;
 }
 
+template <typename T>
+__global__ __launch_bounds__(256) void ups_phase_pack_kernel(const float* __restrict__ src, T* __restrict__ dst, int O, int I) {
+  const int64_t idx = (int64_t)blockIdx.x * 256 + threadIdx.x;
+  if (idx >= (int64_t)16 * O * I) return;
+  const int i = (int)(idx % I);
+  const int tap = (int)((idx / I) & 3);
+  const int o = (int)((idx / ((int64_t)4 * I)) % O);
+  const int ph = (int)(idx / ((int64_t)4 * I * O));
+  const int py = ph >> 1, px = ph & 1, ty = tap >> 1, tx = tap & 1;
+  const int y0 = py ? (ty ? 2 : 0) : (ty ? 1 : 0), y1 = py ? (ty ? 2 : 1) : (ty ? 2 : 0);
+  const int x0 = px ? (tx ? 2 : 0) : (tx ? 1 : 0), x1 = px ? (tx ? 2 : 1) : (tx ? 2 : 0);
+  const float* w = src + ((int64_t)o * I + i) * 9;
+  float v = 0.f;
+  for (int ky = y0; ky <= y1; ++ky)
+    for (int kx = x0; kx <= x1; ++kx) v += w[ky * 3 + kx];
+  dst[idx] = from_f<T>(v);
+}
+
+int launch_pack_ups_phase(int dtype, const float* src, void* dst, int O, int I, hipStream_t s) {
+  const unsigned nb = (unsigned)(((int64_t)16 * O * I + 255) / 256);
+  switch (dtype) {
+    case DT_F16: hipLaunchKernelGGL((ups_phase_pack_kernel<f16>), dim3(nb), dim3(256), 0, s, src, (f16*)dst, O, I); break;
+    case DT_BF16: hipLaunchKernelGGL((ups_phase_pack_kernel<bf16>), dim3(nb), dim3(256), 0, s, src, (bf16*)dst, O, I); break;
+    default: TANGO_FAIL("pack_ups_phase: 16-bit dtypes only");
+  }
+  TANGO_HIP(hipGetLastError());
+  return 0;
+}
+
 
 template <typename T>
 __global__ __launch_bounds__(256) void pointwise_small_kernel(const float* __restrict__ src, const float* __restrict__ W,
diff --git a/tango_amd/csrc/engine.h b/tango_amd/csrc/engine.h
--- a/tango_amd/csrc/engine.h
+++ b/tango_amd/csrc/engine.h
@@ -51,6 +51,7 @@
   int N = 0, K = 0, Cin = 0, taps = 1;
   int64_t Kp = 0;
   bool im2col = false;
+  void* Wph = nullptr;
   void* Wln = nullptr;
   float* bln = nullptr;
   float* wsum = nullptr;
@@ -225,7 +226,7 @@
   void reg_norm(const std::string& p, int C, float eps, WNorm& w);
   void reg_mat(const std::string& wname, int N, int K, WMat& w, bool alloc, int row_off, std::vector<int64_t> shape, bool geglu = false);
   void reg_linear(const std::string& p, int N, int K, WMat& w, bool bias);
-  void reg_conv3x3(const std::string& p, int Cout, int Cin, WMat& w);
+  void reg_conv3x3(const std::string& p, int Cout, int Cin, WMat& w, bool ups_phase = false);
   void reg_conv1x1(const std::string& p, int Cout, int Cin, WMat& w);
   void reg_conv1d(const std::string& p, int Cout, int Cin, int k, WMat& w);
   void reg_convt1d(const std::string& p, int Cin, int Cout, int k, int u, ConvTW& w);
diff --git a/tango_amd/csrc/engine.hip b/tango_amd/csrc/engine.hip
--- a/tango_amd/csrc/engine.hip
+++ b/tango_amd/csrc/engine.hip
@@ -160,6 +160,14 @@
     if (o.residual) { p.R = o.residual->p; p.ldr = o.residual->ld; }
     p.a_act = o.a_act; p.a_slope = o.a_slope; p.e_act = o.e_act; p.e_slope = o.e_slope; p.epi = o.epi;
     p.bias2 = o.bias2; p.bias2_stride = o.bias2_stride; p.step_ptr = o.bias2 ? E.d_step : nullptr;
+    if (ups && w.Wph && gemm_pick_splitk(dt, p) <= 1 && gemm_route(dt, p) == ROUTE_CONV_WIDE && conv_ups_phase_ok(dt, p)) {
+      p.Wph = w.Wph;
+      const int d = dt;
+      char buf[160];
+      snprintf(buf, sizeof buf, "conv3x3up(phase) M=%d N=%d K=%d", p.M, p.N, 4 * p.Cin);
+      push([p, d](hipStream_t s) { return launch_gemm(d, p, s); }, buf, 2.0 * p.M * (double)p.N * 4.0 * p.Cin);
+      return;
+    }
     gemm(p, stride == 2 ? "conv3x3s2" : (ups ? "conv3x3up" : "conv3x3"));
   }
 
@@ -633,7 +641,7 @@
   reg_vec(p + ".bias", Cout, &w.b);
 }
 
-void Engine::reg_conv3x3(const std::string& p, int Cout, int Cin, WMat& w) {
+void Engine::reg_conv3x3(const std::string& p, int Cout, int Cin, WMat& w, bool ups_phase) {
   w.N = Cout;
   w.im2col = ((Cin * esz) % 64) != 0;
   if (w.im2col) {
@@ -646,8 +654,13 @@
   void* W = w.W;
   const int64_t Kp = w.Kp;
   const int d = dt;
-  reg_slot(p + ".weight", {Cout, Cin, 3, 3},
-           [=](const float* src, hipStream_t s) { return launch_pack(d, src, W, Cout, 9, Cin, (int64_t)Cin * 9, 1, 9, Kp, 0, s); });
+  void* Wph = nullptr;
+  if (ups_phase && dt != DT_F32 && !w.im2col) w.Wph = Wph = dmalloc((size_t)16 * Cout * Cin * esz);
+  reg_slot(p + ".weight", {Cout, Cin, 3, 3}, [=](const float* src, hipStream_t s) {
+    TANGO_TRY(launch_pack(d, src, W, Cout, 9, Cin, (int64_t)Cin * 9, 1, 9, Kp, 0, s));
+    if (Wph) TANGO_TRY(launch_pack_ups_phase(d, src, Wph, Cout, Cin, s));
+    return 0;
+  });
   reg_vec(p + ".bias", Cout, &w.b);
 }
 
@@ -817,7 +830,7 @@
     }
     if (i != nl - 1) {
       u.has_us = true;
-      reg_conv3x3(bp + ".upsamplers.0.conv", outc, outc, u.us);
+      reg_conv3x3(bp + ".upsamplers.0.conv", outc, outc, u.us, true);
     }
     prev_out = outc;
   }
diff --git a/tango_amd/csrc/gemm.hip b/tango_amd/csrc/gemm.hip
--- a/tango_amd/csrc/gemm.hip
+++ b/tango_amd/csrc/gemm.hip
@@ -381,6 +381,7 @@
   if (p.wb_rows && route != ROUTE_WIDE && route != ROUTE_DUO) TANGO_FAIL("gemm: per-sample weights are implemented by the 256 x 320 / 256 x 160 GEMMs only");
   if (p.glu_tanh && dtype != DT_F32 && route != ROUTE_WIDE && route != ROUTE_DUO)
     TANGO_FAIL("gemm: the tanh-GELU gate (T5 gated-gelu) is implemented by the fp32 kernels and the 256 x 320 / 256 x 160 GEMMs only");
+  if (p.Wph && route != ROUTE_CONV_WIDE) TANGO_FAIL("gemm: upsampler phase weights are implemented by the 256 x 320 conv only");
   switch (route) {
     case ROUTE_WIDE: return launch_gemm_wide(dtype, p, s);
     case ROUTE_DUO: return launch_gemm_duo(dtype, p, s);
diff --git a/tango_amd/csrc/gemm_wide_device.h b/tango_amd/csrc/gemm_wide_device.h
--- a/tango_amd/csrc/gemm_wide_device.h
+++ b/tango_amd/csrc/gemm_wide_device.h
@@ -24,9 +24,10 @@
   return v;
 }
 
-template <typename T, bool GEGLU, bool RES, bool LN>
+template <typename T, bool GEGLU, bool RES, bool LN, bool UPH = false>
 __device__ __forceinline__ void wide_epilogue(const GemmParams& p, f32x4 (&acc)[10][4], const float (&mean)[4], const float (&rstd)[4],
-                                              const int m_base, const int n_base, const int lane, unsigned char* stage) {
+                                              const int m_base, const int n_base, const int lane, unsigned char* stage, const int phase = 0) {
+  static_assert(!UPH || (!GEGLU && !RES && !LN), "phase rows: plain epilogue only");
   constexpr int TN = 10, NIT = 5;
   constexpr int OC = GEGLU ? 80 : 160;
   constexpr int PITCH = OC * 4 + 16;
@@ -106,7 +107,14 @@
       for (int e = 0; e < 8; ++e) tv[e] = from_f<T>(f[e]);
       u32x4 o;
       __builtin_memcpy(&o, tv, 16);
-      *(u32x4*)(Ob + (int64_t)(m_base + ps * RPP + prow[it]) * ldo + ocol0 + pcol[it]) = o;
+      int64_t orow = m_base + ps * RPP + prow[it];
+      if (UPH) {
+        const int m = (int)orow, hw = p.H * p.Wd;
+        const int bi = m / hw, r = m - bi * hw;
+        const int i = r / p.Wd, j = r - i * p.Wd;
+        orow = ((int64_t)bi * 2 * p.H + 2 * i + (phase >> 1)) * (2 * p.Wd) + 2 * j + (phase & 1);
+      }
+      *(u32x4*)(Ob + orow * ldo + ocol0 + pcol[it]) = o;
     }
     __builtin_amdgcn_wave_barrier();
   }
diff --git a/tango_amd/csrc/ops_abi.hip b/tango_amd/csrc/ops_abi.hip
--- a/tango_amd/csrc/ops_abi.hip
+++ b/tango_amd/csrc/ops_abi.hip
@@ -73,10 +73,8 @@
   return launch_gemm(dt, p, s);
 }
 
-extern "C" {
-
-int tango_op_conv2d(int dt, const float* x, const float* w, const float* bias, float* out, int B, int Cin, int H, int W, int Cout,
-                    int stride, int upsample, void* stream) {
+static int op_conv2d_impl(int dt, const float* x, const float* w, const float* bias, const float* bias2, float* out, int B, int Cin, int H, int W,
+                          int Cout, int stride, int upsample, int phases, void* stream) {
   hipStream_t s = (hipStream_t)stream;
   const size_t esz = dtype_size(dt);
   Scratch sc;
@@ -91,6 +89,7 @@
   TANGO_TRY(launch_nchw_to_nhwc(dt, x, xt, cpad, B, Cin, H * W, 1, 1.0f, s));
   GemmParams p;
   p.bias = bias; p.N = Cout; p.out = ot; p.ldo = Cout;
+  if (bias2) { p.bias2 = bias2; p.bias2_stride = Cout; }
   if (im2col) {
     if (stride != 1 || upsample) TANGO_FAIL("op_conv2d: small-Cin path supports stride 1 only");
     const int64_t Kp = ((9 * Cin + 31) / 32) * 32;
@@ -108,9 +107,37 @@
     TANGO_TRY(launch_pack(dt, w, wt, Cout, 9, Cin, (int64_t)Cin * 9, 1, 9, Kp, 0, s));
     p.A = xt; p.lda = cpad; p.W = wt; p.Kp = Kp; p.M = B * Ho * Wo; p.K = 9 * Cin; p.Cin = Cin;
     p.mode = GATHER_2D; p.H = Ho; p.Wd = Wo; p.Hin = H; p.Win = W; p.stride = stride; p.ups = upsample;
+    const bool ph_ok = upsample == 1 && stride == 1 && phases != 0 && gemm_pick_splitk(dt, p) <= 1 &&
+                       gemm_route(dt, p) == ROUTE_CONV_WIDE && conv_ups_phase_ok(dt, p);
+    if (phases == 1 && !ph_ok) TANGO_FAIL("op_conv2d_ups: the phase form does not take this problem");
+    if (ph_ok) {
+      void* wph = sc.get((size_t)16 * Cout * Cin * esz);
+      if (!wph) TANGO_FAIL("op_conv2d: alloc");
+      TANGO_TRY(launch_pack_ups_phase(dt, w, wph, Cout, Cin, s));
+      p.Wph = wph;
+    }
   }
   TANGO_TRY(run_gemm(dt, p, sc, s));
   TANGO_TRY(launch_nhwc_to_nchw_f32(dt, ot, Cout, out, B, Cout, Ho * Wo, s));
+  TANGO_HIP(hipStreamSynchronize(s));
+  return 0;
+}
+
+extern "C" {
+
+int tango_op_conv2d(int dt, const float* x, const float* w, const float* bias, float* out, int B, int Cin, int H, int W, int Cout,
+                    int stride, int upsample, void* stream) {
+  return op_conv2d_impl(dt, x, w, bias, nullptr, out, B, Cin, H, W, Cout, stride, upsample, -1, stream);
+}
+
+int tango_op_conv2d_ups(int dt, const float* x, const float* w, const float* bias, const float* bias2, float* out, int B, int Cin, int H,
+                        int W, int Cout, int phases, void* stream) {
+  return op_conv2d_impl(dt, x, w, bias, bias2, out, B, Cin, H, W, Cout, 1, 1, phases ? 1 : 0, stream);
+}
+
+int tango_op_pack_ups_phase(int dt, const float* w, void* out, int Cout, int Cin, void* stream) {
+  hipStream_t s = (hipStream_t)stream;
+  TANGO_TRY(launch_pack_ups_phase(dt, w, out, Cout, Cin, s));
   TANGO_HIP(hipStreamSynchronize(s));
   return 0;
 }
diff --git a/tango_amd/csrc/tuning.h b/tango_amd/csrc/tuning.h
--- a/tango_amd/csrc/tuning.h
+++ b/tango_amd/csrc/tuning.h
@@ -47,6 +47,7 @@
   int attn_x8_qb;
   int conv_tall;
   int wide_pipe;
+  bool ups_phases;
   int conv_pipe;
 };
 
@@ -88,6 +89,7 @@
   x.wide_pipe = num("TANGO_WIDE_PIPE", 0);
   x.conv_pipe = num("TANGO_CONV_PIPE", 2);
   x.conv_tall = num("TANGO_CONV_TALL", 0);
+  x.ups_phases = num("TANGO_UPS_PHASES", 1) != 0;
   x.attn_x8_qb = num("TANGO_ATTN_X8_QB", 2);
   x.attn_defer = num("TANGO_ATTN_DEFER", 0);
   x.attn_kdma = num("TANGO_ATTN_KDMA", 1);
diff --git a/tango_amd/weights.py b/tango_amd/weights.py
--- a/tango_amd/weights.py
+++ b/tango_amd/weights.py
@@ -287,3 +287,34 @@
 def iter_synth(shapes: Shapes, seed: int = 1234) -> Iterator[Tuple[str, torch.Tensor]]:
     for k, s in shapes.items():
         yield k, synth_tensor(k, s, seed)
+
+
+UPS_PHASE_TAPS = {(0, 0): (0,), (0, 1): (1, 2), (1, 0): (0, 1), (1, 1): (2,)}
+
+
+def upsample_phase_weights(w: torch.Tensor) -> torch.Tensor:
+    O, I = w.shape[:2]
+    out = torch.zeros(4, O, 2, 2, I, dtype=w.dtype)
+    for py in (0, 1):
+        for px in (0, 1):
+            for ty in (0, 1):
+                for tx in (0, 1):
+                    acc = torch.zeros(O, I, dtype=w.dtype)
+                    for ky in UPS_PHASE_TAPS[(py, ty)]:
+                        for kx in UPS_PHASE_TAPS[(px, tx)]:
+                            acc = acc + w[:, :, ky, kx]
+                    out[2 * py + px, :, ty, tx, :] = acc
+    return out
+
+
+def upsample_phase_conv(x: torch.Tensor, wp: torch.Tensor, bias=None) -> torch.Tensor:
+    import torch.nn.functional as F
+    B, _, H, W = x.shape
+    O = wp.shape[1]
+    out = torch.zeros(B, O, 2 * H, 2 * W, dtype=x.dtype)
+    for py in (0, 1):
+        for px in (0, 1):
+            k = wp[2 * py + px].permute(0, 3, 1, 2).contiguous()
+            xp = F.pad(x, (1 - px, px, 1 - py, py))
+            out[:, :, py::2, px::2] = F.conv2d(xp, k, bias)
+    return out
```

After: 33.07 audio-seconds/s (median of 6 runs). 1.03x the previous value.
